# WeijingShi/Point-GNN

Measured on AMD Instinct MI355X. Metric: KITTI-shaped frames/sec (car_auto_T3 inference: graph build + GNN, 20000 pts/frame, mean E1 602k), higher is better.
Workload: dtype f32

## Files before the change

include/pointgnn_hip.h:

```cpp
#ifndef POINTGNN_HIP_H_
#define POINTGNN_HIP_H_

#include <stddef.h>
#include <stdint.h>

#ifdef __cplusplus
extern "C" {
#endif

#define PGNN_E_INVALID (-1)
#define PGNN_E_WORKSPACE (-2)
#define PGNN_E_UNSUPPORTED (-3)
#define PGNN_E_CAPACITY (-4)
#define PGNN_E_COMM (-5)

int pgnn_version(void);
const char *pgnn_last_error(void);
int pgnn_check_device_pointer(const void *device_ptr);

int pgnn_stream_create_cu_mask(int32_t cu_first, int32_t cu_count,
                               int32_t complement, void **stream_out);
int pgnn_stream_destroy(void *stream);

int pgnn_scatter_max_f32(const float *data, int64_t ld_data,
// ... 319 lines not shown
                                       int32_t num_vertices,
                                       const pgnn_fc_layer *layer_host,
                                       int32_t edges_sorted, float *out,
                                       int64_t ld_out, float *rows_out,
                                       int64_t ld_rows, float *h1_out,
                                       void *stream);

int pgnn_offset_apply(const float *xyz, const float *delta, int64_t ld_delta,
                      int64_t n_rows, const float *wx, float *xyz_out,
                      float *Q, int64_t ld_q, void *stream);

int pgnn_vertex_pre_edge_fwd(const float *h, int64_t ld_h, int32_t c,
                             const float *xyz,
                             const pgnn_fc_layer *offset_layers_host,
                             int32_t n_offset_layers,
                             const pgnn_fc_layer *p_layer_host, const float *wx,
                             int64_t n_vertices, float *P, float *Q,
                             int64_t ld_pq, float *agg, int64_t ld_agg,
                             void *stream);
int pgnn_vertex_pre_edge_fwd_dyn(const float *h, int64_t ld_h, int32_t c,
                                 const float *xyz,
                                 const pgnn_fc_layer *offset_layers_host,
                                 int32_t n_offset_layers,
                                 const pgnn_fc_layer *p_layer_host,
                                 const float *wx, int64_t vertices_cap,
                                 float *P, float *Q, int64_t ld_pq, float *agg,
                                 int64_t ld_agg,
                                 const pgnn_dyn_count *n_vertices,
                                 void *stream);

int pgnn_vertex_update_pre_edge_fwd(
    const float *x, int64_t ld_x, int32_t nx,
    const pgnn_fc_layer *front_layers_host, int32_t n_front,
    const float *residual, int64_t ld_res, float *y, int64_t ld_y, int32_t c,
    const float *xyz, const pgnn_fc_layer *offset_layers_host,
    int32_t n_offset_layers, const pgnn_fc_layer *p_layer_host, const float *wx,
    int64_t n_vertices, float *P, float *Q, int64_t ld_pq, float *agg,
    int64_t ld_agg, void *stream);
int pgnn_vertex_update_pre_edge_fwd_dyn(
    const float *x, int64_t ld_x, int32_t nx,
    const pgnn_fc_layer *front_layers_host, int32_t n_front,
    const float *residual, int64_t ld_res, float *y, int64_t ld_y, int32_t c,
    const float *xyz, const pgnn_fc_layer *offset_layers_host,
    int32_t n_offset_layers, const pgnn_fc_layer *p_layer_host, const float *wx,
    int64_t vertices_cap, float *P, float *Q, int64_t ld_pq, float *agg,
    int64_t ld_agg, const pgnn_dyn_count *n_vertices, void *stream);

int pgnn_mlp2_fwd(const float *x, int64_t ld_x, int32_t nx,
                  const pgnn_fc_layer *front_layers_host, int32_t n_front,
                  const float *residual, int64_t ld_res, float *y, int64_t ld_y,
                  int32_t ny, const pgnn_fc_layer *back_layers_host,
                  int32_t n_back, float *out, int64_t ld_out, int64_t n_rows,
                  void *stream);
int pgnn_mlp2_fwd_dyn(const float *x, int64_t ld_x, int32_t nx,
                      const pgnn_fc_layer *front_layers_host, int32_t n_front,
                      const float *residual, int64_t ld_res, float *y,
                      int64_t ld_y, int32_t ny,
                      const pgnn_fc_layer *back_layers_host, int32_t n_back,
                      float *out, int64_t ld_out, int64_t rows_cap,
                      const pgnn_dyn_count *rows, void *stream);


int pgnn_pack_fc_device(const float *w, const float *b, int32_t k_in,
                        int32_t n_out, int32_t transpose, float *packed,
                        void *stream);

int pgnn_pack_fc_many(const void *jobs_device, int32_t n_jobs,
                      int32_t total_blocks, void *stream);

int pgnn_edge_hidden_fwd(const float *P, const float *Q, int64_t ld_pq,
                         const int32_t *edges, int64_t n_edges, float *H1,
                         void *stream);
int pgnn_edge_hidden_bwd(const float *dH1, int64_t ld, const int32_t *edges,
                         int64_t n_edges, int64_t n_vertices, float *dP,
                         float *dQ, void *stream);
typedef struct pgnn_merge_job {
  const void *src;
  void *dst;
  int64_t n_words;
  int32_t add0, add1;
} pgnn_merge_job;
int pgnn_merge_rows(const pgnn_merge_job *jobs_host, int32_t n_jobs,
                    void *stream);
int pgnn_pool_features_fwd(const float *point_features, int32_t n_feat,
                           const float *point_xyz,
                           const int32_t *keypoint_indices,
                           const int32_t *edges, int64_t n_edges, float *F,
                           void *stream);
int pgnn_pool_features_wide_fwd(const float *point_features,
                                int64_t ld_features, int32_t n_feat,
                                const float *point_xyz,
                                const int32_t *keypoint_indices,
                                const int32_t *edges, int64_t n_edges, float *F,
                                int64_t ld_f, void *stream);
int pgnn_relu_mask_mul(float *dY, const float *Y, int64_t count, void *stream);
int pgnn_scatter_max_bwd_f32(const float *data, int64_t ld_data,
                             const int32_t *seg_ids, int64_t n_rows,
                             int32_t n_cols, int32_t num_segments,
                             const float *out, int64_t ld_out,
                             const float *grad_out, int64_t ld_grad_out,
                             int32_t *tie_count_ws, float *grad_data,
                             int64_t ld_grad_data, int32_t relu_mask,
                             void *stream);
size_t pgnn_segmax_fc_bwd_workspace_bytes(int64_t n_rows, int32_t n_cols,
                                          int32_t num_segments, int32_t k_in);
int pgnn_segmax_fc_bwd_f32(const float *Y, int64_t ld_y,
                           const int32_t *seg_ids, int64_t n_rows,
                           int32_t n_cols, int32_t num_segments,
                           const float *out, int64_t ld_out,
                           const float *grad_out, int64_t ld_go,
                           const float *X, int64_t ld_x, int32_t k_in,
                           const float *WT, int64_t ld_wt, float *dX,
                           int64_t ld_dx, int32_t dx_cols, int32_t mask_x,
                           float *dW, float *db, void *workspace,
                           size_t workspace_bytes, void *stream);
int pgnn_edge_segmax_fc_bwd_f32(const float *Y, int64_t ld_y,
                                const int32_t *edges, const int32_t *dst_ids,
                                int64_t n_edges, int32_t n_cols,
                                int32_t num_vertices, const float *out,
                                int64_t ld_out, const float *grad_out,
                                int64_t ld_go, const float *H1, int64_t ld_h1,
                                const float *P, const float *Q, int32_t k_in,
                                const float *WT, int64_t ld_wt,
                                float *dP, float *dQ, int64_t ld_pq, float *dW,
                                float *db, void *workspace,
                                size_t workspace_bytes, void *stream);
size_t pgnn_weight_grad_workspace_bytes(int32_t k_in, int32_t n_out,
                                        int64_t n_rows);
int pgnn_weight_grad_f32(const float *X, int64_t ld_x, int32_t k_in,
                         const float *dZ, int64_t ld_dz, int32_t n_out,
                         int64_t n_rows, float *dW, float *db,
                         int32_t accumulate, void *workspace,
                         size_t workspace_bytes, void *stream);
size_t pgnn_pool_narrow_bwd_workspace_bytes(int64_t n_rows);
int pgnn_pool_narrow_bwd_f32(const float *feat, const float *act0,
                             const float *act1, const float *dz2,
                             int64_t n_rows, const float *w2t_packed,
                             const float *w1t_packed, int32_t k_in0, float *dW0,
                             float *db0, float *dW1, float *db1, float *dW2,
                             float *db2, int32_t accumulate, void *workspace,
                             size_t workspace_bytes, void *stream);
typedef struct pgnn_wgrad_job {
  const float *X;
  int64_t ld_x;
  const float *dZ;
  int64_t ld_dz;
  int64_t n_rows;
  float *dW;
  float *db;
  int32_t k_in, n_out;
  int32_t accumulate, reserved;
} pgnn_wgrad_job;
size_t pgnn_weight_grad_many_workspace_bytes(const pgnn_wgrad_job *jobs_host,
                                             int32_t n_jobs);
int pgnn_weight_grad_many_f32(const pgnn_wgrad_job *jobs_host, int32_t n_jobs,
                              void *workspace, size_t workspace_bytes,
                              void *stream);
int pgnn_loss_fwd_bwd(const float *logits, int64_t ld_logits,
                      const int32_t *labels, const float *pred_box,
                      int32_t box_len, const float *gt_box, const float *valid,
                      int64_t n_vertices, int32_t num_classes,
                      float cls_grad_scale, float loc_grad_scale,
                      double *sums4, float *dlogits, float *dpred_box,
                      void *stream);
int pgnn_loss_fwd_bwd_counts(const float *logits, int64_t ld_logits,
                             const int32_t *labels, const float *pred_box,
// ... 123 lines not shown
                              int32_t num_classes, int32_t *out_index,
                              int32_t *out_label, int64_t capacity,
                              int32_t *out_count, void *stream);
int pgnn_detection_candidates_dyn(const float *probs, int64_t n_vertices_cap,
                                  const int32_t *n_vertices_dev,
                                  int32_t num_classes, int32_t *out_index,
                                  int32_t *out_label, int64_t capacity,
                                  int32_t *out_count, void *stream);
size_t pgnn_nms_workspace_bytes(int64_t n_boxes);
int pgnn_nms_boxes_3d(const int32_t *class_labels, const float *boxes_3d,
                      const float *scores, const int32_t *attributes,
                      int64_t n_boxes, double overlapped_thres, int32_t mode,
                      float appr_factor, int64_t top_k, void *workspace,
                      size_t workspace_bytes, int32_t *out_labels,
                      float *out_boxes, float *out_scores,
                      int32_t *out_attributes, int32_t *out_count,
                      void *stream);
int pgnn_overlapped_boxes_3d(const float *single_box, const float *boxes_3d,
                             int64_t n_boxes, float appr_factor,
                             double *overlap, void *stream);
int pgnn_overlapped_boxes_3d_raster(const int32_t *single_box_corners,
                                    const int32_t *box_corners, int64_t n_boxes,
                                    double *overlap, void *stream);

int pgnn_assign_box_labels(const float *xyz, int64_t n_points,
                           const double *label_records, int32_t n_records,
                           int32_t *cls_labels, double *boxes_3d,
                           float *valid_boxes, int32_t *owner, void *stream);
int pgnn_assign_box_labels_f64(const double *xyz, int64_t n_points,
                               const double *label_records, int32_t n_records,
                               int32_t *cls_labels, double *boxes_3d,
                               float *valid_boxes, int32_t *owner,
                               void *stream);
int pgnn_box_encode_f64(const int32_t *cls_labels, const float *xyz,
                        const double *boxes, const double *class_table,
                        int32_t n_table, int64_t n_rows, int32_t boxes_per_row,
                        float *encoded, void *stream);
int pgnn_box_encode_f64_xyz64(const int32_t *cls_labels, const double *xyz,
                              const double *boxes, const double *class_table,
                              int32_t n_table, int64_t n_rows,
                              int32_t boxes_per_row, float *encoded,
                              void *stream);

int pgnn_points_affine_f64(double *xyz, int64_t n_points, const double *rot_3x3,
                           const double *shift_3, const int32_t *select,
                           void *stream);
int pgnn_points_in_box_f64(const double *xyz, int64_t n_points,
                           const double *box_record_24, const int32_t *exclude,
                           int32_t *inside, int32_t *count, void *stream);

size_t pgnn_metrics_state_bytes(int32_t n_classes, int32_t n_thresholds);
int pgnn_metrics_update(const float *probs, int64_t ld_probs,
                        const int32_t *labels, int64_t n_rows,
                        int32_t n_classes, int32_t n_thresholds, void *state,
                        void *stream);
int pgnn_metrics_compute(const void *state, int32_t n_classes,
                         int32_t n_thresholds, float *out, void *stream);

size_t pgnn_kitti_ingest_workspace_bytes(int64_t n_points);
int pgnn_kitti_cam_points_in_image(
    const float *velo_points, int64_t n_points, const float *velo_to_cam_3x4,
    const double *cam_to_image_3x3, double image_width, double image_height,
    const uint8_t *image_bgr, int64_t image_rows, int64_t image_cols,
    void *workspace, size_t workspace_bytes, float *out_xyz, float *out_attr,
    int32_t attr_dim, int64_t capacity, int32_t *out_count, void *stream);

size_t pgnn_voxel_average_workspace_bytes(int64_t n_points, int32_t attr_dim);
int pgnn_voxel_average_f32(const float *xyz, const float *attr,
                           int32_t attr_dim, int64_t n_points,
                           const int32_t *n_dev, double voxel_size,
                           void *workspace, size_t workspace_bytes,
                           double *out_xyz, double *out_attr, int32_t *out_lens,
                           int64_t capacity, int32_t *out_count, void *stream);
size_t pgnn_kitti_cam_points_voxel_in_image_workspace_bytes(int64_t n_points);
int pgnn_kitti_cam_points_voxel_in_image(
    const float *velo_points, int64_t n_points, const float *velo_to_cam_3x4,
    const double *cam_to_image_3x3, double image_width, double image_height,
    const uint8_t *image_bgr, int64_t image_rows, int64_t image_cols,
    double voxel_size, void *workspace, size_t workspace_bytes,
    double *out_xyz, double *out_attr, int32_t attr_dim, int64_t capacity,
    int32_t *out_count, void *stream);

int pgnn_set_tunable(const char *key, int value);
int pgnn_set_debug_buffer(void *device_ptr);

#ifdef __cplusplus
}
#endif
#endif
```

point-gnn_amd/_lib.py:

```python
import ctypes
import os

import torch

_HERE = os.path.dirname(os.path.abspath(__file__))
LIB_PATH = os.environ.get("PGNN_LIB") or os.path.join(_HERE, "libpointgnn_hip.so")

c_i32, c_i64, c_f64 = ctypes.c_int32, ctypes.c_int64, ctypes.c_double
c_vp, c_sz, c_u64 = ctypes.c_void_p, ctypes.c_size_t, ctypes.c_uint64

PGNN_MAX_LAYERS = 8


class FcLayer(ctypes.Structure):
    _fields_ = [("packed", c_vp), ("k_in", c_i32), ("n_out", c_i32),
                ("relu_from", c_i32)]


class DynCount(ctypes.Structure):
    _fields_ = [("dev", c_vp), ("hint", c_i64)]


class WgradJob(ctypes.Structure):
    _fields_ = [("X", c_vp), ("ld_x", c_i64), ("dZ", c_vp), ("ld_dz", c_i64),
                ("n_rows", c_i64), ("dW", c_vp), ("db", c_vp), ("k_in", c_i32),
                ("n_out", c_i32), ("accumulate", c_i32), ("reserved", c_i32)]


class MergeJob(ctypes.Structure):
    _fields_ = [("src", c_vp), ("dst", c_vp), ("n_words", c_i64),
                ("add0", c_i32), ("add1", c_i32)]


class PackJob(ctypes.Structure):
    _fields_ = [("w", c_vp), ("b", c_vp), ("dst", c_vp), ("k_in", c_i32),
                ("n_out", c_i32), ("kind", c_i32), ("first_block", c_i32),
                ("ld", c_i32), ("reserved", c_i32)]


TRAIN_MAX_FC, TRAIN_MAX_STAGES, TRAIN_MAX_CLASSES, TRAIN_MAX_LEVELS = 8, 8, 16, 4


class TrainFc(ctypes.Structure):
    _fields_ = [("w_off", c_i64), ("b_off", c_i64), ("k_in", c_i32),
                ("n_out", c_i32)]


class TrainStage(ctypes.Structure):
    _fields_ = [("kind", c_i32), ("graph_level", c_i32), ("n_a", c_i32),
                ("n_b", c_i32), ("n_c", c_i32), ("reserved", c_i32),
                ("a", TrainFc * TRAIN_MAX_FC), ("b", TrainFc * TRAIN_MAX_FC),
                ("c", TrainFc * TRAIN_MAX_FC)]


class TrainModel(ctypes.Structure):
    _fields_ = [("n_stages", c_i32), ("num_classes", c_i32),
                ("box_len", c_i32), ("reserved", c_i32), ("n_params", c_i64),
                ("stages", TrainStage * TRAIN_MAX_STAGES),
                ("cls", TrainFc * 2),
                ("loc", (TrainFc * 3) * TRAIN_MAX_CLASSES)]


class TrainBatch(ctypes.Structure):
    _fields_ = [("input_v", c_vp), ("n_feat", c_i32), ("n_levels", c_i32),
                ("n_vertices", c_i64 * (TRAIN_MAX_LEVELS + 1)),
                ("coords", c_vp * (TRAIN_MAX_LEVELS + 1)),
                ("keypoints", c_vp * TRAIN_MAX_LEVELS),
                ("edges", c_vp * TRAIN_MAX_LEVELS),
                ("n_edges", c_i64 * TRAIN_MAX_LEVELS),
                ("edges_sorted", c_i32 * TRAIN_MAX_LEVELS)]


class PointGnnHipError(RuntimeError):
    pass


_SIGNATURES = {
    "pgnn_version": (c_i32, []),
    "pgnn_last_error": (ctypes.c_char_p, []),
    "pgnn_stream_create_cu_mask": (c_i32, [c_i32, c_i32, c_i32,
                                           ctypes.POINTER(c_vp)]),
    "pgnn_stream_destroy": (c_i32, [c_vp]),
    "pgnn_check_device_pointer": (c_i32, [c_vp]),
    "pgnn_set_tunable": (c_i32, [ctypes.c_char_p, c_i32]),
    "pgnn_set_debug_buffer": (c_i32, [c_vp]),
    "pgnn_scatter_max_f32": (c_i32, [c_vp, c_i64, c_vp, c_i64, c_i32, c_i32,
                                     c_vp, c_i64, c_i32, c_vp]),
    "pgnn_scatter_sum_f32": (c_i32, [c_vp, c_i64, c_vp, c_i64, c_i32, c_i32,
                                     c_vp, c_i64, c_i32, c_vp, c_vp]),
    "pgnn_radius_graph_workspace_bytes": (c_sz, [c_i64, c_i64]),
    "pgnn_radius_graph_count": (c_i32, [c_vp, c_i64, c_vp, c_i64, c_f64, c_vp,
                                        c_vp, c_sz, c_vp, c_vp]),
    "pgnn_radius_graph_fill": (c_i32, [c_vp, c_i64, c_vp, c_i64, c_f64, c_vp,
                                       c_vp, c_sz, c_vp, c_vp, c_i64, c_vp]),
    "pgnn_radius_graph_count_f64": (c_i32, [c_vp, c_i64, c_vp, c_i64, c_f64,
                                            c_vp, c_vp, c_sz, c_vp, c_vp]),
    "pgnn_radius_graph_fill_f64": (c_i32, [c_vp, c_i64, c_vp, c_i64, c_f64,
                                           c_vp, c_vp, c_sz, c_vp, c_vp, c_i64,
                                           c_vp]),
    "pgnn_radius_graph_dyn_workspace_bytes": (c_sz, [c_i64, c_i64]),
    "pgnn_radius_graph_dyn": (c_i32, [c_vp, c_i64, c_vp, c_vp, c_i64, c_vp,
                                      c_f64, c_vp, c_vp, c_sz, c_vp, c_i64,
                                      c_vp, c_vp]),
    "pgnn_radius_graph_dyn_f64": (c_i32, [c_vp, c_i64, c_vp, c_vp, c_i64, c_vp,
                                          c_f64, c_vp, c_vp, c_sz, c_vp, c_i64,
                                          c_vp, c_vp]),
    "pgnn_radius_graph_dyn_grid": (c_i32, [c_vp, c_i64, c_vp, c_i64, c_f64,
                                           c_vp, c_vp, c_sz, c_vp]),
    "pgnn_radius_graph_dyn_grid_f64": (c_i32, [c_vp, c_i64, c_vp, c_i64, c_f64,
                                               c_vp, c_vp, c_sz, c_vp]),
    "pgnn_radius_graph_dyn_query": (c_i32, [c_vp, c_i64, c_vp, c_i64, c_vp,
                                            c_f64, c_vp, c_vp, c_sz, c_vp,
                                            c_i64, c_vp, c_vp]),
    "pgnn_radius_graph_dyn_query_f64": (c_i32, [c_vp, c_i64, c_vp, c_i64, c_vp,
# ... 133 lines not shown
        c_i32, c_vp, c_i64, c_vp, ctypes.POINTER(DynCount),
        ctypes.POINTER(DynCount), c_vp]),
    "pgnn_pack_fc_f16x2_acc": (c_i32, [c_vp, c_vp, c_i32, c_i32, c_vp]),
    "pgnn_point_set_pooling_f16x2_fwd": (c_i32, [
        c_vp, c_i32, c_vp, c_vp, c_vp, c_i64, c_i32, ctypes.POINTER(FcLayer),
        c_i32, c_vp, c_vp, c_i32, c_vp, c_i64, c_vp, c_vp, ctypes.POINTER(DynCount),
        ctypes.POINTER(DynCount), c_vp]),
    "pgnn_offset_apply": (c_i32, [c_vp, c_vp, c_i64, c_i64, c_vp, c_vp, c_vp,
                                  c_i64, c_vp]),
    "pgnn_vertex_pre_edge_fwd": (c_i32, [c_vp, c_i64, c_i32, c_vp,
                                         ctypes.POINTER(FcLayer), c_i32,
                                         ctypes.POINTER(FcLayer), c_vp, c_i64,
                                         c_vp, c_vp, c_i64, c_vp, c_i64,
                                         c_vp]),
    "pgnn_vertex_update_pre_edge_fwd": (c_i32, [
        c_vp, c_i64, c_i32, ctypes.POINTER(FcLayer), c_i32, c_vp, c_i64, c_vp,
        c_i64, c_i32, c_vp, ctypes.POINTER(FcLayer), c_i32,
        ctypes.POINTER(FcLayer), c_vp, c_i64, c_vp, c_vp, c_i64, c_vp, c_i64,
        c_vp]),
    "pgnn_vertex_update_pre_edge_fwd_dyn": (c_i32, [
        c_vp, c_i64, c_i32, ctypes.POINTER(FcLayer), c_i32, c_vp, c_i64, c_vp,
        c_i64, c_i32, c_vp, ctypes.POINTER(FcLayer), c_i32,
        ctypes.POINTER(FcLayer), c_vp, c_i64, c_vp, c_vp, c_i64, c_vp, c_i64,
        ctypes.POINTER(DynCount), c_vp]),
    "pgnn_mlp2_fwd": (c_i32, [
        c_vp, c_i64, c_i32, ctypes.POINTER(FcLayer), c_i32, c_vp, c_i64, c_vp,
        c_i64, c_i32, ctypes.POINTER(FcLayer), c_i32, c_vp, c_i64, c_i64,
        c_vp]),
    "pgnn_mlp2_fwd_dyn": (c_i32, [
        c_vp, c_i64, c_i32, ctypes.POINTER(FcLayer), c_i32, c_vp, c_i64, c_vp,
        c_i64, c_i32, ctypes.POINTER(FcLayer), c_i32, c_vp, c_i64, c_i64,
        ctypes.POINTER(DynCount), c_vp]),
    "pgnn_pack_fc_device": (c_i32, [c_vp, c_vp, c_i32, c_i32, c_i32, c_vp,
                                    c_vp]),
    "pgnn_pack_fc_many": (c_i32, [c_vp, c_i32, c_i32, c_vp]),
    "pgnn_segmax_fc_bwd_workspace_bytes": (c_sz, [c_i64, c_i32, c_i32, c_i32]),
    "pgnn_edge_segmax_fc_bwd_f32": (c_i32, [c_vp, c_i64, c_vp, c_vp, c_i64,
                                            c_i32, c_i32, c_vp, c_i64, c_vp,
                                            c_i64, c_vp, c_i64, c_vp, c_vp,
                                            c_i32, c_vp, c_i64, c_vp, c_vp,
                                            c_i64, c_vp, c_vp, c_vp, c_sz,
                                            c_vp]),
    "pgnn_segmax_fc_bwd_f32": (c_i32, [c_vp, c_i64, c_vp, c_i64, c_i32, c_i32,
                                       c_vp, c_i64, c_vp, c_i64, c_vp, c_i64,
                                       c_i32, c_vp, c_i64, c_vp, c_i64, c_i32,
                                       c_i32, c_vp, c_vp, c_vp, c_sz, c_vp]),
    "pgnn_trainer_create": (c_i32, [ctypes.POINTER(TrainModel),
                                    ctypes.POINTER(c_vp)]),
    "pgnn_trainer_destroy": (c_i32, [c_vp]),
    "pgnn_trainer_images_bytes": (c_sz, [c_vp]),
    "pgnn_trainer_bind": (c_i32, [c_vp, c_vp, c_vp, c_vp, c_sz, c_vp]),
    "pgnn_trainer_repack": (c_i32, [c_vp, c_vp]),
    "pgnn_trainer_workspace_bytes": (c_sz, [c_vp, ctypes.POINTER(TrainBatch)]),
    "pgnn_trainer_forward": (c_i32, [c_vp, ctypes.POINTER(TrainBatch), c_vp,
                                     c_sz, ctypes.POINTER(c_vp),
                                     ctypes.POINTER(c_i64),
                                     ctypes.POINTER(c_vp), c_vp]),
    "pgnn_trainer_backward": (c_i32, [c_vp, ctypes.POINTER(TrainBatch), c_vp,
                                      c_sz, c_vp, c_vp, c_vp]),
    "pgnn_trainer_backward_sync": (c_i32, [c_vp, ctypes.POINTER(TrainBatch),
                                           c_vp, c_sz, c_vp, c_vp, c_vp, c_vp,
                                           c_i64, c_vp]),
    "pgnn_comm_unique_id": (c_i32, [c_vp]),
    "pgnn_comm_init_rank": (c_i32, [c_vp, c_i32, c_i32, ctypes.POINTER(c_vp)]),
    "pgnn_comm_destroy": (c_i32, [c_vp]),
    "pgnn_comm_info": (c_i32, [c_vp, ctypes.POINTER(c_i32),
                               ctypes.POINTER(c_i32), ctypes.POINTER(c_i32)]),
    "pgnn_comm_library": (ctypes.c_char_p, []),
    "pgnn_comm_async_error": (c_i32, [c_vp]),
    "pgnn_allreduce_sum_f32": (c_i32, [c_vp, c_vp, c_i64, c_vp]),
    "pgnn_allreduce_sum_f64": (c_i32, [c_vp, c_vp, c_i64, c_vp]),
    "pgnn_allreduce_step": (c_i32, [c_vp, c_vp, c_i64, c_vp, c_i64, c_vp]),
    "pgnn_broadcast_f32": (c_i32, [c_vp, c_vp, c_i64, c_i32, c_vp]),
    "pgnn_edge_hidden_fwd": (c_i32, [c_vp, c_vp, c_i64, c_vp, c_i64, c_vp,
                                     c_vp]),
    "pgnn_edge_hidden_bwd": (c_i32, [c_vp, c_i64, c_vp, c_i64, c_i64, c_vp,
                                     c_vp, c_vp]),
    "pgnn_pool_features_wide_fwd": (c_i32, [c_vp, c_i64, c_i32, c_vp, c_vp, c_vp,
                                            c_i64, c_vp, c_i64, c_vp]),
    "pgnn_pool_features_fwd": (c_i32, [c_vp, c_i32, c_vp, c_vp, c_vp, c_i64,
                                       c_vp, c_vp]),
    "pgnn_relu_mask_mul": (c_i32, [c_vp, c_vp, c_i64, c_vp]),
    "pgnn_merge_rows": (c_i32, [ctypes.POINTER(MergeJob), c_i32, c_vp]),
    "pgnn_scatter_max_bwd_f32": (c_i32, [c_vp, c_i64, c_vp, c_i64, c_i32,
                                         c_i32, c_vp, c_i64, c_vp, c_i64, c_vp,
                                         c_vp, c_i64, c_i32, c_vp]),
    "pgnn_weight_grad_workspace_bytes": (c_sz, [c_i32, c_i32, c_i64]),
    "pgnn_weight_grad_f32": (c_i32, [c_vp, c_i64, c_i32, c_vp, c_i64, c_i32,
                                     c_i64, c_vp, c_vp, c_i32, c_vp, c_sz,
                                     c_vp]),
    "pgnn_weight_grad_many_workspace_bytes": (c_sz,
                                              [ctypes.POINTER(WgradJob),
                                               c_i32]),
    "pgnn_weight_grad_many_f32": (c_i32, [ctypes.POINTER(WgradJob), c_i32,
                                          c_vp, c_sz, c_vp]),
    "pgnn_pool_narrow_bwd_workspace_bytes": (c_sz, [c_i64]),
    "pgnn_pool_narrow_bwd_f32": (c_i32, [c_vp, c_vp, c_vp, c_vp, c_i64, c_vp,
                                         c_vp, c_i32, c_vp, c_vp, c_vp, c_vp,
                                         c_vp, c_vp, c_i32, c_vp, c_sz, c_vp]),
    "pgnn_loss_fwd_bwd": (c_i32, [c_vp, c_i64, c_vp, c_vp, c_i32, c_vp, c_vp,
                                  c_i64, c_i32, ctypes.c_float, ctypes.c_float,
                                  c_vp, c_vp, c_vp, c_vp]),
    "pgnn_loss_fwd_bwd_counts": (c_i32, [c_vp, c_i64, c_vp, c_vp, c_i32, c_vp,
                                         c_vp, c_i64, c_i32, ctypes.c_double,
                                         ctypes.c_double, c_vp, c_vp, c_vp,
                                         c_vp, c_vp]),
    "pgnn_loss_fwd_bwd_ex": (c_i32, [c_vp, c_i64, c_vp, c_vp, c_i32, c_vp, c_vp,
                                     c_i64, c_i32, ctypes.c_float,
                                     ctypes.c_float, c_vp, ctypes.c_double,
                                     ctypes.c_double, c_i32, ctypes.c_float,
                                     ctypes.c_float, c_vp, c_vp, c_vp, c_vp,
                                     c_vp]),
    "pgnn_loss_fwd_bwd_sel": (c_i32, [c_vp, c_i64, c_vp, c_vp, c_i32, c_vp,
                                      c_vp, c_i64, c_i32, ctypes.c_float,
                                      ctypes.c_float, c_vp, ctypes.c_double,
                                      ctypes.c_double, c_i32, ctypes.c_float,
                                      ctypes.c_float, c_vp, c_vp, c_vp,
                                      ctypes.c_float, c_vp, c_vp, c_vp, c_vp,
                                      c_vp, c_vp]),
    "pgnn_topk_mask_workspace_bytes": (c_sz, [c_i64]),
    "pgnn_topk_mask_f32": (c_i32, [c_vp, c_i64, c_i64, c_vp, c_vp, c_sz, c_vp]),
    "pgnn_sgd_step": (c_i32, [c_vp, c_vp, c_vp, c_i64, ctypes.c_float,
                              ctypes.c_float, ctypes.c_float, c_vp]),
    "pgnn_optimizer_step": (c_i32, [c_i32, c_vp, c_vp, c_vp, c_vp, c_vp, c_i64] +
                            [ctypes.c_float] * 6 + [c_vp]),
    "pgnn_l1_norm": (c_i32, [c_vp, c_vp, c_i64, c_vp, c_vp]),
    "pgnn_box_decode_f32": (c_i32, [c_vp, c_vp, c_vp, c_vp, c_i32, c_i64,
                                    c_i32, c_vp, c_vp]),
    "pgnn_box_encode_f32": (c_i32, [c_vp, c_vp, c_vp, c_vp, c_i32, c_i64,
                                    c_i32, c_vp, c_vp]),
    "pgnn_detection_candidates": (c_i32, [c_vp, c_i64, c_i32, c_vp, c_vp,
                                          c_i64, c_vp, c_vp]),
    "pgnn_detection_candidates_dyn": (c_i32, [c_vp, c_i64, c_vp, c_i32, c_vp,
                                              c_vp, c_i64, c_vp, c_vp]),
    "pgnn_nms_workspace_bytes": (c_sz, [c_i64]),
    "pgnn_nms_boxes_3d": (c_i32, [c_vp, c_vp, c_vp, c_vp, c_i64,
                                  c_f64, c_i32, ctypes.c_float, c_i64,
                                  c_vp, c_sz, c_vp, c_vp, c_vp, c_vp, c_vp,
                                  c_vp]),
    "pgnn_overlapped_boxes_3d": (c_i32, [c_vp, c_vp, c_i64, ctypes.c_float,
                                         c_vp, c_vp]),
    "pgnn_overlapped_boxes_3d_raster": (c_i32, [c_vp, c_vp, c_i64, c_vp,
                                                c_vp]),
    "pgnn_assign_box_labels": (c_i32, [c_vp, c_i64, c_vp, c_i32, c_vp, c_vp,
                                       c_vp, c_vp, c_vp]),
    "pgnn_assign_box_labels_f64": (c_i32, [c_vp, c_i64, c_vp, c_i32, c_vp,
                                           c_vp, c_vp, c_vp, c_vp]),
    "pgnn_box_encode_f64": (c_i32, [c_vp, c_vp, c_vp, c_vp, c_i32, c_i64,
                                    c_i32, c_vp, c_vp]),
    "pgnn_box_encode_f64_xyz64": (c_i32, [c_vp, c_vp, c_vp, c_vp, c_i32, c_i64,
                                          c_i32, c_vp, c_vp]),
    "pgnn_points_affine_f64": (c_i32, [c_vp, c_i64, c_vp, c_vp, c_vp, c_vp]),
    "pgnn_points_in_box_f64": (c_i32, [c_vp, c_i64, c_vp, c_vp, c_vp, c_vp,
                                       c_vp]),
    "pgnn_kitti_ingest_workspace_bytes": (c_sz, [c_i64]),
    "pgnn_kitti_cam_points_in_image": (c_i32, [c_vp, c_i64, c_vp, c_vp, c_f64,
                                               c_f64, c_vp, c_i64, c_i64, c_vp,
                                               c_sz, c_vp, c_vp, c_i32, c_i64,
                                               c_vp, c_vp]),
    "pgnn_voxel_average_workspace_bytes": (c_sz, [c_i64, c_i32]),
    "pgnn_voxel_average_f32": (c_i32, [c_vp, c_vp, c_i32, c_i64, c_vp, c_f64,
                                       c_vp, c_sz, c_vp, c_vp, c_vp, c_i64,
                                       c_vp, c_vp]),
    "pgnn_kitti_cam_points_voxel_in_image_workspace_bytes": (c_sz, [c_i64]),
    "pgnn_kitti_cam_points_voxel_in_image": (
        c_i32, [c_vp, c_i64, c_vp, c_vp, c_f64, c_f64, c_vp, c_i64, c_i64,
# ... 32 lines not shown
    if _lib is not None:
        return _lib
    if not os.path.exists(LIB_PATH) and not os.environ.get("PGNN_LIB"):
        _build_missing()
    if not os.path.exists(LIB_PATH):
        raise PointGnnHipError(
            "libpointgnn_hip.so not found at %s -- the HIP extension is "
            "required (no CPU fallback); run `python -m pointgnn_amd.build`"
            % LIB_PATH)
    lib = ctypes.CDLL(LIB_PATH)
    for name, (res, args) in _SIGNATURES.items():
        fn = getattr(lib, name)
        fn.restype = res
        fn.argtypes = args
    _lib = lib
    for kv in filter(None, os.environ.get("PGNN_TUNE", "").split(",")):
        k, v = kv.split("=")
        check(lib.pgnn_set_tunable(k.strip().encode(), int(v)),
              "PGNN_TUNE " + kv)
    return lib


E_INVALID = -1
E_WORKSPACE = -2
E_UNSUPPORTED = -3
AGG_MAX, AGG_SUM, AGG_MEAN = 0, 1, 2


def check(rc, what=""):
    if rc != 0:
        msg = load().pgnn_last_error()
        raise PointGnnHipError("%s failed (code %d): %s" % (
            what or "pgnn call", rc, msg.decode() if msg else "?"))


_SCHED_WS = {}
SCHED_WS_INTS = 64


def sched_ws(device=None):
    import torch
    dev = torch.device("cuda", torch.cuda.current_device()) \
        if device is None or device.index is None else device
    key = (dev.index, torch.cuda.current_stream(dev).cuda_stream)
    t = _SCHED_WS.get(key)
    if t is None:
        t = _SCHED_WS[key] = torch.zeros(SCHED_WS_INTS, dtype=torch.int32,
                                         device=dev)
    return t


def stream_ptr():
    return ctypes.c_void_p(torch.cuda.current_stream().cuda_stream)


def ptr(t):
    if t is None:
        return ctypes.c_void_p(0)
    return ctypes.c_void_p(t.data_ptr())


class DeviceCount(object):
    __slots__ = ("dev", "hint", "frame")

    def __init__(self, dev, hint=0, frame=None):
        self.dev = dev
        self.hint = int(hint)
        self.frame = frame

    def arg(self):
        return ctypes.byref(DynCount(self.dev.data_ptr(), self.hint))


def tag_count(t, count):
    if count is not None:
        t._pgnn_count = count
    return t


def count_of(t):
    return getattr(t, "_pgnn_count", None) if t is not None else None


def set_tunable(key, value):
    check(load().pgnn_set_tunable(key.encode(), int(value)), "pgnn_set_tunable")
```

point-gnn_amd/csrc/gnn.hip:

```cpp
#include "mlp_engine.h"
#include "edge_ws.h"
#include "edge_ws_split.h"
#include "pool_ws.h"
#include "pool_split.h"
#include "pool_ws_f16.h"

namespace pgnn {
int g_mlp_blocks_per_cu = 4;
int g_edge_msub = 0;
int g_pool_msub = 0;
int g_mlp_pool_pct = 12;
int g_ws_xcds = 8;
int g_ws_prio = 1;
int g_f16_pool = 1;
int g_b16_force = 0;
int g_ws_pool_pct = 0;
int g_ws_chunk = 2;
int g_ws_balance = 1;
int g_ws_reserve = 0;
void *g_mlp_ts = nullptr;
int g_mlp_debug = 0;
}

namespace {
using namespace pgnn;

enum { PRO_ROWS = 0, PRO_POOL = 1, PRO_EDGE = 2,
       PRO_POOL_R3 = 3 };
constexpr bool is_pool(int pro) { return pro == PRO_POOL || pro == PRO_POOL_R3; }
constexpr bool is_pool_reg(int pro) { return pro == PRO_POOL_R3; }
constexpr int kMaxRegisterRuns = 6;

struct RowsArgs {
  const float *x;
  int64_t ldx;
  int nx;
  const float *x2;
  int64_t ldx2;
  int nx2;
  const float *res;
  int64_t ldres;
  float *y;
  int64_t ldy;
  int res_gate;
  float *mid[PGNN_MAX_LAYERS - 1];
  const float *gate[PGNN_MAX_LAYERS - 1];
};
struct PoolArgs {
  const float *feat;
  int nfeat;
  const float *xyz;
  const int32_t *kp;
  const int32_t *edges;
  int reg_hidden;
};
struct EdgeArgs {
  const float *P;
  const float *Q;
  int64_t ldpq;
  const int32_t *edges;
};
struct SegArgs {
  float *out;
  int64_t ldo;
  int num_segments;
  int sorted;
};

__host__ __device__ inline int ints_bytes(int rows) {
  return ((2 * rows + 2) * 4 + 15) / 16 * 16;
}

struct CarryState {
  int id;
  int left_closed;
};

__device__ __forceinline__ CarryState carry_after(unsigned long long starts,
                                                  int myd, int d_before,
                                                  int d_after, const SegArgs &sa,
                                                  CarryState cs, bool keep_open) {
  CarryState out = {-1, 0};
// ... 19 lines not shown
  const int myd = lane < ROWS ? dst[lane + 1] : -2;
  const int prevd = lane < ROWS ? dst[lane] : -2;
  const unsigned long long starts =
      __ballot(lane < ROWS && (lane == 0 || myd != prevd));
  const int d_before = dst[0], d_after = dst[ROWS + 1];
  for (int c = threadIdx.x; c < ncols; c += 256) {
    const float *col = stT + c * ROWS;
    const int sw = c & SWZ;
    v4f x[G];
#pragma unroll
    for (int g = 0; g < G; ++g)
      x[g] = *reinterpret_cast<const v4f *>(col + ((g ^ sw) << 2));
    unsigned long long rem = starts;
    while (rem) {
      const int r = __builtin_ctzll(rem);
      rem &= rem - 1;
      const int re = rem ? __builtin_ctzll(rem) : ROWS;
      const int d = __builtin_amdgcn_readlane(myd, r);
      if (d >= 0 && d < sa.num_segments) {
        bool left_closed = (r > 0) || (d_before != d);
        const bool merge = sa.sorted && r == 0 && cs.id == d;
        if (merge) left_closed = cs.left_closed != 0;
        const bool right_closed = (re < ROWS) || (d_after != d);
        const bool defer = sa.sorted && !right_closed && keep_open;
        const bool whole = sa.sorted && left_closed && right_closed;
        const int g0 = r >> 2, g1 = (re - 1) >> 2;
        float m = kFloatLowest;
#pragma unroll
        for (int g = 0; g < G; ++g) {
          if (g > g0 && g < g1) {
            m = fmaxf(fmaxf(m, x[g][0]), fmaxf(x[g][1], fmaxf(x[g][2], x[g][3])));
          } else if (g == g0 || g == g1) {
#pragma unroll
            for (int i = 0; i < 4; ++i) {
              const int row = 4 * g + i;
              if (row >= r && row < re) m = fmaxf(m, x[g][i]);
            }
          }
        }
        if (merge) m = fmaxf(m, carry[col0 + c]);
        if (defer) {
          carry[col0 + c] = m;
        } else {
          float *o = sa.out + (int64_t)d * sa.ldo + col0 + c;
          if (whole)
            *o = m;
          else
            atomic_max_f32(o, m + 0.0f);
        }
      }
    }
  }
  return carry_after(starts, myd, d_before, d_after, sa, cs, keep_open);
}

template <int ROWS>
__device__ __forceinline__ void consume_rows(const float *__restrict__ stage,
                                             int ld, int64_t row0, int rows_valid,
                                             int col0, int ncols,
                                             const RowsArgs &ra) {
  const int total = rows_valid * ncols;
  for (int idx = threadIdx.x; idx < total; idx += blockDim.x) {
    const int r = idx / ncols, c = idx - r * ncols;
    float v = stage[r * ld + c];
    if (ra.res) {
      const float a = ra.res[(row0 + r) * ra.ldres + col0 + c];
      v = ra.res_gate ? (a > 0.0f ? v : 0.0f) : v + a;
    }
    ra.y[(row0 + r) * ra.ldy + col0 + c] = v;
  }
}

__device__ __forceinline__ int opaque_lane(int lane_id) {
  int lane;
  asm volatile("v_mov_b32 %0, %1" : "=v"(lane) : "v"(lane_id));
  return lane;
}

constexpr int kRowSteps = 10;

__device__ __forceinline__ void consume_rows16(const float *__restrict__ stage,
                                               int ld, int64_t row0,
                                               int rows_valid, int col0,
                                               int ncols, const RowsArgs &ra) {
  const int r = threadIdx.x >> 5, c0 = threadIdx.x & 31;
  const int64_t row = row0 + (r < rows_valid ? r : rows_valid - 1);
  float add[kRowSteps];
  if (ra.res) {
    const float *__restrict__ rr = ra.res + row * ra.ldres + col0;
#pragma unroll
    for (int j = 0; j < kRowSteps; ++j) {
      const int c = c0 + 32 * j;
      add[j] = rr[c < ncols ? c : ncols - 1];
    }
  }
  float *__restrict__ yr = ra.y + row * ra.ldy + col0;
#pragma unroll
  for (int j = 0; j < kRowSteps; ++j) {
    const int c = c0 + 32 * j;
    if (r < rows_valid && c < ncols) {
      float v = stage[r * ld + c];
      if (ra.res) v = ra.res_gate ? (add[j] > 0.0f ? v : 0.0f) : v + add[j];
      yr[c] = v;
    }
  }
}

__device__ __forceinline__ void tap_rows16(float *tile, int ld, int64_t row0,
                                           int rows_valid, int ncols,
                                           const float *__restrict__ gate,
                                           float *__restrict__ mid) {
  const int r = threadIdx.x >> 5, c0 = threadIdx.x & 31;
  const int64_t row = row0 + (r < rows_valid ? r : rows_valid - 1);
  for (int cb = 0; cb < ncols; cb += 32 * kRowSteps) {
    const int left = ncols - cb;
    float g[kRowSteps];
    if (gate) {
      const float *__restrict__ gr = gate + row * ncols + cb;
#pragma unroll
      for (int j = 0; j < kRowSteps; ++j) {
        const int c = c0 + 32 * j;
        g[j] = gr[c < left ? c : left - 1];
      }
    }
    float *tr = tile + r * ld + cb;
    float *__restrict__ mr = mid ? mid + row * ncols + cb : nullptr;
#pragma unroll
    for (int j = 0; j < kRowSteps; ++j) {
      const int c = c0 + 32 * j;
      if (c < left) {
        float v = tr[c];
        if (gate) {
          v = g[j] > 0.0f ? v : 0.0f;
          tr[c] = v;
        }
        if (mr && r < rows_valid) mr[c] = v;
      }
    }
  }
  if (gate) __syncthreads();
}

__device__ __forceinline__ void load_rows16(const float *__restrict__ x,
                                            int64_t ldx, int nx, float *tile,
                                            int ld0, int kc, int64_t row0,
                                            int rows_valid) {
  const int r = threadIdx.x >> 5, c0 = threadIdx.x & 31;
  const float *__restrict__ xr =
      x + (row0 + (r < rows_valid ? r : rows_valid - 1)) * ldx;
  for (int cb = 0; cb < kc; cb += 32 * kRowSteps) {
    float v[kRowSteps];
#pragma unroll
    for (int j = 0; j < kRowSteps; ++j) {
      const int c = cb + c0 + 32 * j;
      v[j] = xr[c < nx ? c : nx - 1];
    }
#pragma unroll
    for (int j = 0; j < kRowSteps; ++j) {
      const int c = cb + c0 + 32 * j;
      if (c < kc) tile[r * ld0 + c] = (r < rows_valid && c < nx) ? v[j] : 0.0f;
    }
  }
}

template <int MSUB, int PRO>
__global__ __launch_bounds__(256, 2) void fused_mlp_kernel(
    ChainDev chain, int64_t n_rows, RowsArgs ra, PoolArgs pa, EdgeArgs ea,
    SegArgs sa, int stage_off ,
    int dbg, long long *ts ,
    int32_t *sched ,
    int64_t n_static ,
    const int32_t *n_dev ,
    int dyn_pool_pct ) {
  constexpr int ROWS = 16 * MSUB;
  if (n_dev) {
    const int64_t nd = *n_dev;
    n_rows = nd < n_rows ? nd : n_rows;
  }
#ifndef PGNN_DIAG
  dbg &= ~7;
#endif
  extern __shared__ __attribute__((aligned(16))) char smem[];
  int *dst = reinterpret_cast<int *>(smem);
  float *part = reinterpret_cast<float *>(dst + ROWS + 2);
  if (MSUB == 4 && threadIdx.x < 48) part[threadIdx.x] = kFloatLowest;
  float *carry = reinterpret_cast<float *>(smem + ints_bytes(ROWS));
  float *tile = carry + 16 * chain.l[chain.n - 1].nt;
  float *stage = stage_off >= 0 ? tile + stage_off : tile;
  const int lane = threadIdx.x & 63;
  const int wave = __builtin_amdgcn_readfirstlane(threadIdx.x >> 6);
  const int64_t n_tiles = (n_rows + ROWS - 1) / ROWS;
  const int ld0 = lds_ld(16 * chain.l[0].kq);

  if (n_dev) {
    if (sched && n_tiles >= 6 * (int64_t)gridDim.x)
      n_static = n_tiles - n_tiles * dyn_pool_pct / 100;
    else
      sched = nullptr;
  }
  if (!sched) n_static = n_tiles;
  const int64_t tq = n_static / gridDim.x, trem = n_static % gridDim.x;
  const int64_t tile_first =
      blockIdx.x * tq + (blockIdx.x < trem ? blockIdx.x : trem);
  int64_t tile_last = tile_first + tq + (blockIdx.x < trem ? 1 : 0);
  __shared__ int s_claim;
  CarryState cs = {-1, 0};
  int nxt_s = 0, nxt_d = -1, nxt_k = 0;
  bool fresh = true;
  int tile_seq = 0;
  for (int64_t tile_id = tile_first;; ++tile_id, ++tile_seq) {
    if (tile_id >= tile_last) {
      if (tile_id >= n_tiles || !sched) break;
      if (threadIdx.x == 0)
        s_claim = __hip_atomic_fetch_add(&sched[0], 1, __ATOMIC_RELAXED,
                                         __HIP_MEMORY_SCOPE_AGENT);
      __syncthreads();
      tile_id = n_static + __builtin_amdgcn_readfirstlane(s_claim);
      if (tile_id >= n_tiles) break;
      tile_last = tile_id + 1;
      cs.id = -1;
      cs.left_closed = 0;
      fresh = true;
    }
    const int64_t row0 = tile_id * ROWS;
    const int rows_valid =
        (int)((n_rows - row0 < ROWS) ? (n_rows - row0) : ROWS);
    long long *tsp = nullptr;
    if (ts && tile_seq < 32 && threadIdx.x == 0) {
      tsp = ts + ((int64_t)blockIdx.x * 32 + tile_seq) * 8;
      tsp[0] = __builtin_readcyclecounter();
// ... 387 lines not shown
int make_plan(const pgnn_fc_layer *layers, int32_t n_layers, int first_k,
              Plan &p) {
  PGNN_REQUIRE(layers && n_layers >= 1 && n_layers <= PGNN_MAX_LAYERS,
               PGNN_E_INVALID, "mlp: 1..PGNN_MAX_LAYERS layers required");
  p.chain.n = n_layers;
  int prev_nt = -1;
  int max_ld = 0;
  for (int i = 0; i < n_layers; ++i) {
    const pgnn_fc_layer &l = layers[i];
    PGNN_REQUIRE(l.packed && l.k_in > 0 && l.n_out > 0, PGNN_E_INVALID,
                 "mlp: bad layer");
    LayerDev &d = p.chain.l[i];
    d.wp = l.packed;
    d.kq = (l.k_in + 15) / 16;
    d.nt = (l.n_out + 15) / 16;
    d.relu_from = l.relu_from;
    if (i == 0) {
      PGNN_REQUIRE(first_k <= l.k_in, PGNN_E_INVALID,
                   "mlp: input wider than first layer");
    } else {
      PGNN_REQUIRE(d.kq == prev_nt, PGNN_E_INVALID,
                   "mlp: layer widths do not chain");
    }
    if (i + 1 < n_layers)
      PGNN_REQUIRE(d.nt <= kMaxTilesPerPass, PGNN_E_UNSUPPORTED,
                   "mlp: hidden width > 320 not supported");
    prev_nt = d.nt;
    const int ld_in = lds_ld(16 * d.kq);
    if (ld_in > max_ld) max_ld = ld_in;
    if (i + 1 < n_layers || d.nt <= kMaxTilesPerPass) {
      const int ld_out = lds_ld(16 * d.nt);
      if (ld_out > max_ld) max_ld = ld_out;
    }
  }
  p.tile_floats_per_row = max_ld;
  p.stage_cols =
      p.chain.l[n_layers - 1].nt > kMaxTilesPerPass ? 16 * kMaxTilesPerPass : 0;
  return 0;
}

size_t plan_lds_bytes(const Plan &p, int rows) {
  size_t floats = (size_t)rows * p.tile_floats_per_row;
  floats += 16 * (size_t)p.chain.l[p.chain.n - 1].nt;
  if (p.stage_cols) floats += (size_t)rows * lds_ld(p.stage_cols);
  return ints_bytes(rows) + floats * 4;
}

template <int MSUB, int PRO>
int launch_fused(const Plan &p, int64_t n_rows, const RowsArgs &ra,
                 const PoolArgs &pa, const EdgeArgs &ea, const SegArgs &sa,
                 hipStream_t stream, int32_t *sched = nullptr,
                 const int32_t *n_dev = nullptr) {
  constexpr int ROWS = 16 * MSUB;
  const size_t lds = plan_lds_bytes(p, ROWS);
  PGNN_REQUIRE(lds <= 160 * 1024, PGNN_E_UNSUPPORTED,
               "mlp: layer too wide for the LDS tile");
  auto kern = fused_mlp_kernel<MSUB, PRO>;
  const int64_t n_tiles = (n_rows + ROWS - 1) / ROWS;
  int per_cu = (int)((160 * 1024) / lds);
  if (per_cu > g_mlp_blocks_per_cu) per_cu = g_mlp_blocks_per_cu;
  if (per_cu < 1) per_cu = 1;
  int64_t grid = (int64_t)stream_cu_count(stream) * per_cu;
  if (grid > n_tiles) grid = n_tiles;
  int64_t n_static = n_tiles;
  if (g_mlp_ts || g_mlp_pool_pct <= 0 || (!n_dev && n_tiles < 6 * grid))
    sched = nullptr;
  if (sched) n_static = n_tiles - n_tiles * g_mlp_pool_pct / 100;
  PGNN_HIP((hipError_t)arm_sched(sched, stream));
  const int stage_off = p.stage_cols ? ROWS * p.tile_floats_per_row : -1;
  if (g_mlp_debug & 16) {
    int nb = -1;
    hipError_t e = hipOccupancyMaxActiveBlocksPerMultiprocessor(
        &nb, reinterpret_cast<const void *>(kern), 256, lds);
    fprintf(stderr, "[pgnn] fused<%d,%d> lds=%zu per_cu=%d occupancy_api=%d (%d) grid=%lld tiles=%lld\n",
            MSUB, PRO, lds, per_cu, nb, (int)e, (long long)grid, (long long)n_tiles);
  }
  return launch_lds(kern, dim3((unsigned)grid), dim3(256), lds, stream, p.chain,
                    n_rows, ra, pa, ea, sa, stage_off, g_mlp_debug,
                    (long long *)g_mlp_ts, sched, n_static, n_dev,
                    g_mlp_pool_pct);
}

constexpr int kRowsWaves = 8;

template <bool TAPS>
__global__ __launch_bounds__(64 * kRowsWaves) void rows_mlp_kernel(
    ChainDev chain, int64_t n_rows, RowsArgs ra, int stage_off,
    const int32_t *n_dev ) {
  constexpr int ROWS = 16, NW = kRowsWaves;
  if (n_dev) {
    const int64_t nd = *n_dev;
    n_rows = nd < n_rows ? nd : n_rows;
  }
  extern __shared__ __attribute__((aligned(16))) char smem[];
  float *tile = reinterpret_cast<float *>(smem);
  float *stage = stage_off >= 0 ? tile + stage_off : tile;
  const int lane_id = threadIdx.x & 63;
  const int wave = __builtin_amdgcn_readfirstlane(threadIdx.x >> 6);
  const int64_t n_tiles = (n_rows + ROWS - 1) / ROWS;
  const int ld0 = lds_ld(16 * chain.l[0].kq);
  for (int64_t tile_id = blockIdx.x; tile_id < n_tiles; tile_id += gridDim.x) {
    const int lane = opaque_lane(lane_id);
    const int64_t row0 = tile_id * ROWS;
    const int rows_valid =
        (int)((n_rows - row0 < ROWS) ? (n_rows - row0) : ROWS);
    const int kc = 16 * chain.l[0].kq;
    KrowPre pre;
    krow_prefetch(chain.l[0], 0, wave, lane, pre);
    if (ra.nx2 == 0) {
      static_assert(64 * NW == 32 * ROWS, "one 32-thread group per row");
      load_rows16(ra.x, ra.ldx, ra.nx, tile, ld0, kc, row0, rows_valid);
    } else {
    for (int idx = threadIdx.x; idx < ROWS * kc; idx += 64 * NW) {
      const int r = idx / kc, c = idx - r * kc;
      float v = 0.0f;
      if (r < rows_valid) {
        if (c < ra.nx)
          v = ra.x[(row0 + r) * ra.ldx + c];
        else if (c < ra.nx + ra.nx2)
          v = ra.x2[(row0 + r) * ra.ldx2 + (c - ra.nx)];
      }
      tile[r * ld0 + c] = v;
    }
    }
    __syncthreads();
    for (int li = 0; li + 1 < chain.n; ++li) {
      const LayerDev &L = chain.l[li];
      krow_pass(tile, lds_ld(16 * L.kq), tile, lds_ld(16 * L.nt), L, 0, wave,
                lane, pre, true, chain.l[li + 1], 0);
      if constexpr (TAPS)
        tap_rows16(tile, lds_ld(16 * L.nt), row0, rows_valid, 16 * L.nt,
                   ra.gate[li], ra.mid[li]);
    }
    const LayerDev &L = chain.l[chain.n - 1];
    const int ld_in = lds_ld(16 * L.kq);
    for (int t0 = 0; t0 < L.nt; t0 += kMaxTilesPerPass) {
      int tiles = L.nt - t0;
      if (tiles > kMaxTilesPerPass) tiles = kMaxTilesPerPass;
      const int ncols = 16 * tiles;
      const int ld_st = lds_ld(ncols);
      const bool more = t0 + kMaxTilesPerPass < L.nt;
      krow_pass(tile, ld_in, stage, ld_st, L, t0, wave, lane, pre, more, L,
                t0 + kMaxTilesPerPass);
      consume_rows16(stage, ld_st, row0, rows_valid, 16 * t0, ncols, ra);
      __syncthreads();
    }
  }
}

template <bool TAPS = false>
int launch_rows8(const Plan &p, int64_t n_rows, const RowsArgs &ra,
                 hipStream_t stream, const int32_t *n_dev = nullptr,
                 int64_t grid_tiles = 0 ) {
  const size_t lds = plan_lds_bytes(p, 16);
  PGNN_REQUIRE(lds <= 160 * 1024, PGNN_E_UNSUPPORTED,
               "mlp: layer too wide for the LDS tile");
  const int64_t n_tiles = (n_rows + 15) / 16;
  const int stage_off = p.stage_cols ? 16 * p.tile_floats_per_row : -1;
  return launch_lds(rows_mlp_kernel<TAPS>,
                    dim3((unsigned)(grid_tiles > 0 ? grid_tiles : n_tiles)),
                    dim3(64 * kRowsWaves), lds, stream, p.chain, n_rows, ra,
                    stage_off, n_dev);
}

int fill_lowest(float *out, int64_t count, hipStream_t stream) {
  PGNN_HIP(hipMemsetD32Async((hipDeviceptr_t)out, (int)kFloatLowestBits,
// ... 679 lines not shown
    const pgnn_dyn_count *n_edges, const pgnn_dyn_count *num_vertices,
    int32_t aggregation, void *workspace, size_t workspace_bytes,
    void *stream_) {
  PGNN_GUARD_BEGIN
  PGNN_REQUIRE(n_edges && n_edges->dev && num_vertices && num_vertices->dev,
               PGNN_E_INVALID, "edge_mlp_agg_dyn: null count");
  return edge_agg_impl(P, Q, ld_pq, width, edges, edges_cap, vertices_cap, layers,
                       n_layers, edges_sorted, out, ld_out, sched_ws, aggregation,
                       workspace, workspace_bytes, (hipStream_t)stream_,
                       dyn_of(n_edges), dyn_of(num_vertices), true, nullptr);
  PGNN_GUARD_END
}

extern "C" int pgnn_point_set_pooling_agg_workspace_bytes(
    const pgnn_fc_layer *layers, int32_t n_layers, int32_t n_feat,
    int64_t edges_cap, int64_t edges_hint, int32_t keypoints_cap,
    int32_t aggregation, int32_t capacity_form, void *stream_, size_t *bytes) {
  PGNN_GUARD_BEGIN
  PGNN_REQUIRE(bytes && layers, PGNN_E_INVALID,
               "pooling_agg_workspace_bytes: bad arguments");
  const int64_t n_sel =
      (capacity_form && edges_hint > 0 && edges_hint < edges_cap) ? edges_hint
                                                                  : edges_cap;
  return pooling_agg_impl(nullptr, n_feat, nullptr, nullptr, nullptr, n_sel,
                          keypoints_cap, layers, n_layers, 0, nullptr, 0, nullptr,
                          aggregation, nullptr, 0, (hipStream_t)stream_,
                          dyn_of(nullptr), dyn_of(nullptr), capacity_form != 0,
                          bytes);
  PGNN_GUARD_END
}

extern "C" int pgnn_point_set_pooling_agg_fwd(
    const float *point_features, int32_t n_feat, const float *point_xyz,
    const int32_t *keypoint_indices, const int32_t *edges, int64_t n_edges,
    int32_t num_keypoints, const pgnn_fc_layer *layers, int32_t n_layers,
    int32_t edges_sorted, float *out, int64_t ld_out, int32_t *sched_ws,
    int32_t aggregation, void *workspace, size_t workspace_bytes,
    void *stream_) {
  PGNN_GUARD_BEGIN
  return pooling_agg_impl(point_features, n_feat, point_xyz, keypoint_indices,
                          edges, n_edges, num_keypoints, layers, n_layers,
                          edges_sorted, out, ld_out, sched_ws, aggregation,
                          workspace, workspace_bytes, (hipStream_t)stream_,
                          dyn_of(nullptr), dyn_of(nullptr), false, nullptr);
  PGNN_GUARD_END
}

extern "C" int pgnn_point_set_pooling_agg_fwd_dyn(
    const float *point_features, int32_t n_feat, const float *point_xyz,
    const int32_t *keypoint_indices, const int32_t *edges, int64_t edges_cap,
    int32_t keypoints_cap, const pgnn_fc_layer *layers, int32_t n_layers,
    int32_t edges_sorted, float *out, int64_t ld_out, int32_t *sched_ws,
    const pgnn_dyn_count *n_edges, const pgnn_dyn_count *num_keypoints,
    int32_t aggregation, void *workspace, size_t workspace_bytes,
    void *stream_) {
  PGNN_GUARD_BEGIN
  PGNN_REQUIRE(n_edges && n_edges->dev && num_keypoints && num_keypoints->dev,
               PGNN_E_INVALID, "pooling_agg_dyn: null count");
  return pooling_agg_impl(point_features, n_feat, point_xyz, keypoint_indices,
                          edges, edges_cap, keypoints_cap, layers, n_layers,
                          edges_sorted, out, ld_out, sched_ws, aggregation,
                          workspace, workspace_bytes, (hipStream_t)stream_,
                          dyn_of(n_edges), dyn_of(num_keypoints), true, nullptr);
  PGNN_GUARD_END
}

namespace {

struct PreEdgeArgs {
  const float *h;
  int64_t ld_h;
  int c;
  const float *xyz;
  const float *wx;
  int64_t n;
  const int32_t *n_dev;
  float *P, *Q;
  int64_t ld_pq;
  float *agg;
  int64_t ld_agg;
  int ld_tile, ld_scratch;
};

__device__ __forceinline__ void pre_edge_tail(const ChainDev &off,
                                              const LayerDev &pl,
                                              const PreEdgeArgs &a, float *tile,
                                              float *scratch, float *stage,
                                              int64_t row0, int rows_valid,
                                              int wave, int lane, KrowPre &pre) {
  const float *delta = nullptr;
  int ld_delta = 0;
  for (int li = 0; li < off.n; ++li) {
    const LayerDev &L = off.l[li];
    const float *in = li == 0 ? tile : scratch;
    const int ld_in = li == 0 ? a.ld_tile : lds_ld(16 * L.kq);
    krow_pass(in, ld_in, scratch, lds_ld(16 * L.nt), L, 0, wave, lane, pre,
              true, li + 1 < off.n ? off.l[li + 1] : pl, 0);
    delta = scratch;
    ld_delta = lds_ld(16 * L.nt);
  }
  {
    const int r = threadIdx.x >> 5, c0 = threadIdx.x & 31;
    const int ldq = (int)a.ld_pq;
    const int64_t row = row0 + (r < rows_valid ? r : rows_valid - 1);
    float x0 = a.xyz[row * 3], x1 = a.xyz[row * 3 + 1], x2 = a.xyz[row * 3 + 2];
    float w0[kRowSteps], w1[kRowSteps], w2[kRowSteps];
#pragma unroll
    for (int j = 0; j < kRowSteps; ++j) {
      const int c = c0 + 32 * j;
      const int cc = c < ldq ? c : ldq - 1;
      w0[j] = a.wx[cc];
      w1[j] = a.wx[ldq + cc];
      w2[j] = a.wx[2 * ldq + cc];
    }
    if (delta) {
      x0 = x0 + delta[r * ld_delta];
      x1 = x1 + delta[r * ld_delta + 1];
      x2 = x2 + delta[r * ld_delta + 2];
    }
    float *__restrict__ qr = a.Q + row * a.ld_pq;
#pragma unroll
    for (int j = 0; j < kRowSteps; ++j) {
      const int c = c0 + 32 * j;
      if (r < rows_valid && c < ldq)
        qr[c] = (x0 * w0[j] + x1 * w1[j]) + x2 * w2[j];
    }
  }
  const int ld_st = lds_ld(16 * pl.nt);
  krow_pass(tile, a.ld_tile, stage, ld_st, pl, 0, wave, lane, pre, false, pl, 0);
  RowsArgs ra = {};
  ra.y = a.P;
  ra.ldy = a.ld_pq;
  consume_rows16(stage, ld_st, row0, rows_valid, 0, 16 * pl.nt, ra);
}

template <bool STRIDE>
__global__ __launch_bounds__(64 * kRowsWaves) void vertex_pre_edge_kernel(
    ChainDev off, LayerDev pl, PreEdgeArgs a) {
  constexpr int ROWS = 16;
  extern __shared__ __attribute__((aligned(16))) char smem[];
  float *tile = reinterpret_cast<float *>(smem);
  float *scratch = tile + ROWS * a.ld_tile;
  float *stage = scratch + ROWS * a.ld_scratch;
  const int lane_id = threadIdx.x & 63;
  const int wave = __builtin_amdgcn_readfirstlane(threadIdx.x >> 6);
  int64_t n_rows = a.n;
  if (a.n_dev) {
    const int64_t nd = *a.n_dev;
    n_rows = nd < n_rows ? nd : n_rows;
  }
  for (int64_t row0 = (int64_t)blockIdx.x * ROWS; row0 < n_rows;
       row0 += STRIDE ? (int64_t)gridDim.x * ROWS : n_rows) {
    const int lane = opaque_lane(lane_id);
  const int rows_valid =
      (int)((n_rows - row0 < ROWS) ? (n_rows - row0) : ROWS);
  const int kc = 16 * pl.kq;
  KrowPre pre;
  krow_prefetch(off.n > 0 ? off.l[0] : pl, 0, wave, lane, pre);
  {
    static_assert(64 * kRowsWaves == 32 * ROWS, "one 32-thread group per row");
    const int r = threadIdx.x >> 5, c0 = threadIdx.x & 31;
    const int64_t rowc = row0 + (r < rows_valid ? r : rows_valid - 1);
    const float *__restrict__ hr = a.h + rowc * a.ld_h;
    const float *__restrict__ xr = a.xyz + rowc * 3;
    for (int cb = 0; cb < kc; cb += 32 * kRowSteps) {
      float v[kRowSteps];
#pragma unroll
      for (int j = 0; j < kRowSteps; ++j) {
        const int c = cb + c0 + 32 * j;
        const int d = c - a.c;
        const float hv = hr[c < a.c ? c : a.c - 1];
        const float xv = xr[d < 0 ? 0 : (d > 2 ? 2 : d)];
        v[j] = c < a.c ? hv : xv;
      }
#pragma unroll
      for (int j = 0; j < kRowSteps; ++j) {
        const int c = cb + c0 + 32 * j;
        if (c < kc)
          tile[r * a.ld_tile + c] =
              (r < rows_valid && c < a.c + 3) ? v[j] : 0.0f;
      }
    }
  }
  if (a.agg) {
    for (int idx = threadIdx.x; idx < rows_valid * (int)a.ld_agg; idx += 64 * kRowsWaves)
      a.agg[row0 * a.ld_agg + idx] = kFloatLowest;
  }
  __syncthreads();
  pre_edge_tail(off, pl, a, tile, scratch, stage, row0, rows_valid, wave, lane,
                pre);
  if (STRIDE) __syncthreads();
  }
}

struct FrontArgs {
  const float *x;
  int64_t ldx;
  int nx;
  const float *res;
  int64_t ldres;
  float *y;
  int64_t ldy;
  int ld_buf;
  int ld_stage;
  long long *ts;
};

__device__ __forceinline__ void front_chain(const ChainDev &front, float *tile,
                                            float *stage, int ld_stage,
                                            int wave, int lane, KrowPre &pre,
                                            const LayerDev after,
                                            long long *tsw, int &n_stamp) {
  for (int li = 0; li + 1 < front.n; ++li) {
    const LayerDev &L = front.l[li];
    krow_pass(tile, lds_ld(16 * L.kq), tile, lds_ld(16 * L.nt), L, 0, wave,
              lane, pre, true, front.l[li + 1], 0);
    if (tsw && n_stamp < 14) {
      const long long cyc = __builtin_readcyclecounter();
      if (threadIdx.x == 0) tsw[n_stamp] = cyc;
      ++n_stamp;
    }
  }
  const LayerDev &L = front.l[front.n - 1];
  krow_pass(tile, lds_ld(16 * L.kq), stage, ld_stage, L, 0, wave, lane, pre,
            true, after, 0);
}

template <bool STRIDE>
__global__ __launch_bounds__(64 * kRowsWaves) void vertex_update_pre_edge_kernel(
    ChainDev front, FrontArgs f, ChainDev off, LayerDev pl, PreEdgeArgs a) {
  constexpr int ROWS = 16;
  static_assert(64 * kRowsWaves == 32 * ROWS, "one 32-thread group per row");
  extern __shared__ __attribute__((aligned(16))) char smem[];
  float *tile = reinterpret_cast<float *>(smem);
  float *scratch = tile + ROWS * f.ld_buf;
  float *stage = scratch + ROWS * a.ld_scratch;
  const int lane_id = threadIdx.x & 63;
  const int wave = __builtin_amdgcn_readfirstlane(threadIdx.x >> 6);
  int64_t n_rows = a.n;
  if (a.n_dev) {
    const int64_t nd = *a.n_dev;
    n_rows = nd < n_rows ? nd : n_rows;
  }
  const int kc0 = 16 * front.l[0].kq;
  const int ncols_y = 16 * front.l[front.n - 1].nt;
  const int kc = 16 * pl.kq;
  long long *tsw = f.ts ? f.ts + (int64_t)blockIdx.x * 16 : nullptr;
  int n_stamp = 0;
  auto stamp = [&]() {
    if (tsw && n_stamp < 15) {
      __builtin_amdgcn_sched_barrier(0);
      const long long cyc = __builtin_readcyclecounter();
      if (threadIdx.x == 0) tsw[n_stamp] = cyc;
      ++n_stamp;
      __builtin_amdgcn_sched_barrier(0);
    }
  };
  if (tsw && threadIdx.x == 0) tsw[15] = __builtin_amdgcn_s_memrealtime();
  for (int64_t row0 = (int64_t)blockIdx.x * ROWS; row0 < n_rows;
       row0 += STRIDE ? (int64_t)gridDim.x * ROWS : n_rows) {
    const int lane = opaque_lane(lane_id);
    const int rows_valid =
        (int)((n_rows - row0 < ROWS) ? (n_rows - row0) : ROWS);
    stamp();
    KrowPre pre;
    krow_prefetch(front.l[0], 0, wave, lane, pre);
    load_rows16(f.x, f.ldx, f.nx, tile, lds_ld(kc0), kc0, row0, rows_valid);
    if (a.agg) {
      for (int idx = threadIdx.x; idx < rows_valid * (int)a.ld_agg;
           idx += 64 * kRowsWaves)
        a.agg[row0 * a.ld_agg + idx] = kFloatLowest;
    }
    __syncthreads();
    stamp();
    front_chain(front, tile, stage, f.ld_stage, wave, lane, pre,
                off.n > 0 ? off.l[0] : pl, tsw, n_stamp);
    stamp();
    {
      const int r = threadIdx.x >> 5, c0 = threadIdx.x & 31;
      const int64_t row = row0 + (r < rows_valid ? r : rows_valid - 1);
      float add[kRowSteps];
      if (f.res) {
        const float *__restrict__ rr = f.res + row * f.ldres;
#pragma unroll
        for (int j = 0; j < kRowSteps; ++j) {
          const int c = c0 + 32 * j;
          add[j] = rr[c < ncols_y ? c : ncols_y - 1];
        }
      }
      const float xv0 = a.xyz[row * 3], xv1 = a.xyz[row * 3 + 1],
                  xv2 = a.xyz[row * 3 + 2];
      float *__restrict__ yr = f.y + row * f.ldy;
#pragma unroll
      for (int j = 0; j < kRowSteps; ++j) {
        const int c = c0 + 32 * j;
        if (c < kc) {
          float v = 0.0f;
          if (r < rows_valid) {
            if (c < ncols_y) {
              float sv = stage[r * f.ld_stage + c];
              if (f.res) sv += add[j];
              yr[c] = sv;
              if (c < a.c) v = sv;
            }
            const int d = c - a.c;
            if (d >= 0 && d < 3) v = d == 0 ? xv0 : (d == 1 ? xv1 : xv2);
          }
          tile[r * a.ld_tile + c] = v;
        }
      }
    }
    __syncthreads();
    stamp();
    pre_edge_tail(off, pl, a, tile, scratch, stage, row0, rows_valid, wave, lane,
                  pre);
    stamp();
    if (STRIDE) __syncthreads();
  }
  if (tsw && threadIdx.x == 0) tsw[14] = __builtin_amdgcn_s_memrealtime();
}

template <bool STRIDE>
__global__ __launch_bounds__(64 * kRowsWaves) void vertex_mlp2_kernel(
    ChainDev front, FrontArgs f, ChainDev back, RowsArgs out, int64_t n_rows,
    const int32_t *n_dev) {
  constexpr int ROWS = 16;
  extern __shared__ __attribute__((aligned(16))) char smem[];
  float *tile = reinterpret_cast<float *>(smem);
  float *stage = tile + ROWS * f.ld_buf;
  const int lane_id = threadIdx.x & 63;
  const int wave = __builtin_amdgcn_readfirstlane(threadIdx.x >> 6);
  if (n_dev) {
    const int64_t nd = *n_dev;
    n_rows = nd < n_rows ? nd : n_rows;
  }
  const int kc0 = 16 * front.l[0].kq;
  const int ncols_y = 16 * front.l[front.n - 1].nt;
  const int kcb = 16 * back.l[0].kq;
  const int ld_b = lds_ld(kcb);
  for (int64_t row0 = (int64_t)blockIdx.x * ROWS; row0 < n_rows;
       row0 += STRIDE ? (int64_t)gridDim.x * ROWS : n_rows) {
    const int lane = opaque_lane(lane_id);
    const int rows_valid =
        (int)((n_rows - row0 < ROWS) ? (n_rows - row0) : ROWS);
    KrowPre pre;
    krow_prefetch(front.l[0], 0, wave, lane, pre);
    load_rows16(f.x, f.ldx, f.nx, tile, lds_ld(kc0), kc0, row0, rows_valid);
    __syncthreads();
    int no_stamp = 0;
    front_chain(front, tile, stage, f.ld_stage, wave, lane, pre, back.l[0],
                nullptr, no_stamp);
    const int kmax = kcb > ncols_y ? kcb : ncols_y;
    {
      const int r = threadIdx.x >> 5, c0 = threadIdx.x & 31;
      const int64_t row = row0 + (r < rows_valid ? r : rows_valid - 1);
      float add[kRowSteps];
      if (f.res) {
        const float *__restrict__ rr = f.res + row * f.ldres;
#pragma unroll
        for (int j = 0; j < kRowSteps; ++j) {
          const int c = c0 + 32 * j;
          add[j] = rr[c < ncols_y ? c : ncols_y - 1];
        }
      }
      float *__restrict__ yr = f.y + row * f.ldy;
#pragma unroll
      for (int j = 0; j < kRowSteps; ++j) {
        const int c = c0 + 32 * j;
        if (c < kmax) {
          float v = 0.0f;
          if (r < rows_valid && c < ncols_y) {
            float sv = stage[r * f.ld_stage + c];
            if (f.res) sv += add[j];
            yr[c] = sv;
            if (c < out.nx) v = sv;
          }
          if (c < kcb) tile[r * ld_b + c] = v;
        }
      }
    }
    __syncthreads();
    for (int li = 0; li + 1 < back.n; ++li) {
      const LayerDev &L = back.l[li];
      krow_pass(tile, lds_ld(16 * L.kq), tile, lds_ld(16 * L.nt), L, 0, wave,
                lane, pre, true, back.l[li + 1], 0);
    }
    const LayerDev &L = back.l[back.n - 1];
    const int ld_st = lds_ld(16 * L.nt);
    krow_pass(tile, lds_ld(16 * L.kq), stage, ld_st, L, 0, wave, lane, pre,
              false, L, 0);
    consume_rows16(stage, ld_st, row0, rows_valid, 0, 16 * L.nt, out);
    if (STRIDE) __syncthreads();
  }
}

}

namespace {
int plan_pre_edge(const char *name, int32_t c, const float *xyz,
                  const pgnn_fc_layer *offset_layers, int32_t n_offset_layers,
                  const pgnn_fc_layer *p_layer, const float *wx,
                  int64_t n_vertices, float *P, float *Q, int64_t ld_pq,
                  float *agg, int64_t ld_agg, const Dyn &dk, int kq_max,
                  ChainDev &off, LayerDev &pl, PreEdgeArgs &a) {
  const auto msg = [name](const char *what) { return std::string(name) + what; };
  Plan pp;
  int rc = make_plan(p_layer, 1, c + 3, pp);
  if (rc) return rc;
  pl = pp.chain.l[0];
  PGNN_REQUIRE(p_layer->k_in == c + 3 && pl.nt <= kMaxTilesPerPass &&
                   ld_pq == 16 * pl.nt,
               PGNN_E_INVALID,
               msg(": P layer must be [c+3 -> n], ld_pq = padded n").c_str());
  PGNN_REQUIRE(kq_max == 0 || pl.kq <= kq_max, PGNN_E_UNSUPPORTED,
               msg(": more than 317 features").c_str());
  off = {};
  int scratch_ld = lds_ld(16);
  if (n_offset_layers > 0) {
    Plan po;
    rc = make_plan(offset_layers, n_offset_layers, c, po);
    if (rc) return rc;
    off = po.chain;
    PGNN_REQUIRE(offset_layers[0].k_in == c &&
                     offset_layers[n_offset_layers - 1].n_out >= 3 &&
                     off.l[0].kq <= pl.kq &&
                     off.l[n_offset_layers - 1].nt <= kMaxTilesPerPass,
                 PGNN_E_INVALID,
                 msg(": offset chain must be [c -> ... -> 3]").c_str());
    for (int i = 0; i < n_offset_layers; ++i) {
      const int ld = lds_ld(16 * off.l[i].nt);
      if (ld > scratch_ld) scratch_ld = ld;
      if (i > 0 && lds_ld(16 * off.l[i].kq) > scratch_ld)
        scratch_ld = lds_ld(16 * off.l[i].kq);
    }
  }
  a.c = c;
  a.xyz = xyz;
  a.wx = wx;
  a.n = n_vertices;
  a.n_dev = dk.dev;
  a.P = P;
  a.Q = Q;
  a.ld_pq = ld_pq;
  a.agg = agg;
  a.ld_agg = ld_agg;
  a.ld_tile = lds_ld(16 * pl.kq);
  a.ld_scratch = scratch_ld;
  return 0;
}

int pre_edge_impl(
    const float *h, int64_t ld_h, int32_t c, const float *xyz,
    const pgnn_fc_layer *offset_layers, int32_t n_offset_layers,
    const pgnn_fc_layer *p_layer, const float *wx, int64_t n_vertices, float *P,
    float *Q, int64_t ld_pq, float *agg, int64_t ld_agg, hipStream_t stream,
    const Dyn &dk) {
  PGNN_REQUIRE(n_vertices >= 0 && c > 0 && ld_h >= c && n_offset_layers >= 0 &&
                   n_offset_layers <= PGNN_MAX_LAYERS && p_layer,
               PGNN_E_INVALID, "vertex_pre_edge: bad argument");
  if (n_vertices == 0) return 0;
  PGNN_REQUIRE(h && xyz && wx && P && Q && (!agg || ld_agg > 0), PGNN_E_INVALID,
               "vertex_pre_edge: null pointer");
  ChainDev off;
  LayerDev pl;
  PreEdgeArgs a;
  const int rc = plan_pre_edge("vertex_pre_edge", c, xyz, offset_layers,
                               n_offset_layers, p_layer, wx, n_vertices, P, Q,
                               ld_pq, agg, ld_agg, dk, 0, off, pl, a);
  if (rc) return rc;
  a.h = h;
  a.ld_h = ld_h;
  const size_t lds =
      (size_t)16 * (a.ld_tile + a.ld_scratch + lds_ld(16 * pl.nt)) * 4;
  PGNN_REQUIRE(lds <= 160 * 1024, PGNN_E_UNSUPPORTED,
               "vertex_pre_edge: layer too wide for the LDS tile");
  return launch_lds(
      dk.dev ? vertex_pre_edge_kernel<true> : vertex_pre_edge_kernel<false>,
      dim3((unsigned)dyn_grid_tiles(dk, n_vertices)), dim3(64 * kRowsWaves), lds,
      stream, off, pl, a);
}
}

namespace {
int plan_front(const float *x, int64_t ld_x, int32_t nx,
               const pgnn_fc_layer *front_layers, int32_t n_front,
               const float *residual, int64_t ld_res, float *y, int64_t ld_y,
               Plan &pf, FrontArgs &f) {
  PGNN_REQUIRE(x && y && nx > 0 && ld_x >= nx, PGNN_E_INVALID,
               "fused vertex stage: bad front input");
  int rc = make_plan(front_layers, n_front, nx, pf);
  if (rc) return rc;
  const int nt_last = pf.chain.l[n_front - 1].nt;
  PGNN_REQUIRE(nt_last <= kMaxTilesPerPass, PGNN_E_UNSUPPORTED,
               "fused vertex stage: front chain wider than 320");
  PGNN_REQUIRE(ld_y >= 16 * nt_last && (!residual || ld_res >= 16 * nt_last),
               PGNN_E_INVALID,
               "fused vertex stage: ld_y / ld_res < padded front width");
  f.x = x;
  f.ldx = ld_x;
  f.nx = nx;
  f.res = residual;
  f.ldres = ld_res;
  f.y = y;
  f.ldy = ld_y;
  f.ld_buf = pf.tile_floats_per_row;
  f.ld_stage = lds_ld(16 * nt_last);
  f.ts = (long long *)g_mlp_ts;
  return 0;
}

int update_pre_edge_impl(
    const float *x, int64_t ld_x, int32_t nx, const pgnn_fc_layer *front_layers,
    int32_t n_front, const float *residual, int64_t ld_res, float *y,
    int64_t ld_y, int32_t c, const float *xyz,
    const pgnn_fc_layer *offset_layers, int32_t n_offset_layers,
    const pgnn_fc_layer *p_layer, const float *wx, int64_t n_vertices, float *P,
    float *Q, int64_t ld_pq, float *agg, int64_t ld_agg, hipStream_t stream,
    const Dyn &dk) {
  PGNN_REQUIRE(n_vertices >= 0 && c > 0 && n_offset_layers >= 0 &&
                   n_offset_layers <= PGNN_MAX_LAYERS && p_layer,
               PGNN_E_INVALID, "vertex_update_pre_edge: bad argument");
  if (n_vertices == 0) return 0;
  PGNN_REQUIRE(xyz && wx && P && Q && (!agg || ld_agg > 0) && agg != x,
               PGNN_E_INVALID, "vertex_update_pre_edge: null / aliased pointer");
  PGNN_REQUIRE(expected(dk, n_vertices) <= 32 * (int64_t)device_cu_count(),
               PGNN_E_UNSUPPORTED, "vertex_update_pre_edge: too many rows");
  Plan pf;
  FrontArgs f;
  int rc = plan_front(x, ld_x, nx, front_layers, n_front, residual, ld_res, y,
                      ld_y, pf, f);
  if (rc) return rc;
  PGNN_REQUIRE(16 * pf.chain.l[n_front - 1].nt >= c &&
                   16 * pf.chain.l[n_front - 1].nt < c + 16,
               PGNN_E_INVALID,
               "vertex_update_pre_edge: front chain must produce c features");
  ChainDev off;
  LayerDev pl;
  PreEdgeArgs a;
  rc = plan_pre_edge("vertex_update_pre_edge", c, xyz, offset_layers,
                     n_offset_layers, p_layer, wx, n_vertices, P, Q, ld_pq, agg,
                     ld_agg, dk, kMaxTilesPerPass, off, pl, a);
  if (rc) return rc;
  a.h = nullptr;
  a.ld_h = 0;
  if (f.ld_buf < a.ld_tile) f.ld_buf = a.ld_tile;
  if (f.ld_stage < lds_ld(16 * pl.nt)) f.ld_stage = lds_ld(16 * pl.nt);
  const size_t lds = (size_t)16 * (f.ld_buf + a.ld_scratch + f.ld_stage) * 4;
  PGNN_REQUIRE(lds <= 160 * 1024, PGNN_E_UNSUPPORTED,
               "vertex_update_pre_edge: layers too wide for the LDS tile");
  return launch_lds(dk.dev ? vertex_update_pre_edge_kernel<true>
                           : vertex_update_pre_edge_kernel<false>,
                    dim3((unsigned)dyn_grid_tiles(dk, n_vertices)),
                    dim3(64 * kRowsWaves), lds, stream, pf.chain, f, off, pl, a);
}

int mlp2_impl(const float *x, int64_t ld_x, int32_t nx,
              const pgnn_fc_layer *front_layers, int32_t n_front,
              const float *residual, int64_t ld_res, float *y, int64_t ld_y,
              int32_t ny, const pgnn_fc_layer *back_layers, int32_t n_back,
              float *out, int64_t ld_out, int64_t n_rows, hipStream_t stream,
              const Dyn &dk) {
  PGNN_REQUIRE(n_rows >= 0 && ny > 0, PGNN_E_INVALID, "mlp2: bad sizes");
  if (n_rows == 0) return 0;
  PGNN_REQUIRE(out, PGNN_E_INVALID, "mlp2: null output");
  PGNN_REQUIRE(expected(dk, n_rows) <= 32 * (int64_t)device_cu_count(),
               PGNN_E_UNSUPPORTED, "mlp2: too many rows for the 16-row kernel");
  Plan pf;
  FrontArgs f;
  int rc = plan_front(x, ld_x, nx, front_layers, n_front, residual, ld_res, y,
                      ld_y, pf, f);
  if (rc) return rc;
  PGNN_REQUIRE(ny <= 16 * pf.chain.l[n_front - 1].nt, PGNN_E_INVALID,
               "mlp2: ny wider than the front chain's output");
  Plan pb;
  rc = make_plan(back_layers, n_back, ny, pb);
  if (rc) return rc;
  const int nt_out = pb.chain.l[n_back - 1].nt;
  PGNN_REQUIRE(nt_out <= kMaxTilesPerPass &&
                   pb.chain.l[0].kq <= kMaxTilesPerPass,
               PGNN_E_UNSUPPORTED, "mlp2: back chain wider than 320");
  PGNN_REQUIRE(ld_out >= 16 * nt_out, PGNN_E_INVALID,
               "mlp2: ld_out < padded output width");
  if (f.ld_buf < pb.tile_floats_per_row) f.ld_buf = pb.tile_floats_per_row;
  if (f.ld_stage < lds_ld(16 * nt_out)) f.ld_stage = lds_ld(16 * nt_out);
  RowsArgs ro = {};
  ro.nx = ny;
  ro.y = out;
  ro.ldy = ld_out;
  const size_t lds = (size_t)16 * (f.ld_buf + f.ld_stage) * 4;
  PGNN_REQUIRE(lds <= 160 * 1024, PGNN_E_UNSUPPORTED,
               "mlp2: layers too wide for the LDS tile");
  return launch_lds(dk.dev ? vertex_mlp2_kernel<true> : vertex_mlp2_kernel<false>,
                    dim3((unsigned)dyn_grid_tiles(dk, n_rows)),
                    dim3(64 * kRowsWaves), lds, stream, pf.chain, f, pb.chain,
                    ro, n_rows, dk.dev);
}
}

extern "C" int pgnn_vertex_update_pre_edge_fwd(
    const float *x, int64_t ld_x, int32_t nx, const pgnn_fc_layer *front_layers,
    int32_t n_front, const float *residual, int64_t ld_res, float *y,
    int64_t ld_y, int32_t c, const float *xyz,
    const pgnn_fc_layer *offset_layers, int32_t n_offset_layers,
    const pgnn_fc_layer *p_layer, const float *wx, int64_t n_vertices, float *P,
    float *Q, int64_t ld_pq, float *agg, int64_t ld_agg, void *stream_) {
  PGNN_GUARD_BEGIN
  return update_pre_edge_impl(x, ld_x, nx, front_layers, n_front, residual,
                              ld_res, y, ld_y, c, xyz, offset_layers,
                              n_offset_layers, p_layer, wx, n_vertices, P, Q,
                              ld_pq, agg, ld_agg, (hipStream_t)stream_,
                              dyn_of(nullptr));
  PGNN_GUARD_END
}

extern "C" int pgnn_vertex_update_pre_edge_fwd_dyn(
    const float *x, int64_t ld_x, int32_t nx, const pgnn_fc_layer *front_layers,
    int32_t n_front, const float *residual, int64_t ld_res, float *y,
    int64_t ld_y, int32_t c, const float *xyz,
    const pgnn_fc_layer *offset_layers, int32_t n_offset_layers,
    const pgnn_fc_layer *p_layer, const float *wx, int64_t vertices_cap,
    float *P, float *Q, int64_t ld_pq, float *agg, int64_t ld_agg,
    const pgnn_dyn_count *n_vertices, void *stream_) {
  PGNN_GUARD_BEGIN
  PGNN_REQUIRE(n_vertices && n_vertices->dev, PGNN_E_INVALID,
               "vertex_update_pre_edge_dyn: null count");
  return update_pre_edge_impl(x, ld_x, nx, front_layers, n_front, residual,
                              ld_res, y, ld_y, c, xyz, offset_layers,
                              n_offset_layers, p_layer, wx, vertices_cap, P, Q,
                              ld_pq, agg, ld_agg, (hipStream_t)stream_,
                              dyn_of(n_vertices));
  PGNN_GUARD_END
}

extern "C" int pgnn_mlp2_fwd(const float *x, int64_t ld_x, int32_t nx,
                             const pgnn_fc_layer *front_layers, int32_t n_front,
                             const float *residual, int64_t ld_res, float *y,
                             int64_t ld_y, int32_t ny,
                             const pgnn_fc_layer *back_layers, int32_t n_back,
                             float *out, int64_t ld_out, int64_t n_rows,
                             void *stream_) {
  PGNN_GUARD_BEGIN
  return mlp2_impl(x, ld_x, nx, front_layers, n_front, residual, ld_res, y,
                   ld_y, ny, back_layers, n_back, out, ld_out, n_rows,
                   (hipStream_t)stream_, dyn_of(nullptr));
  PGNN_GUARD_END
}

extern "C" int pgnn_mlp2_fwd_dyn(const float *x, int64_t ld_x, int32_t nx,
                                 const pgnn_fc_layer *front_layers,
                                 int32_t n_front, const float *residual,
                                 int64_t ld_res, float *y, int64_t ld_y,
                                 int32_t ny, const pgnn_fc_layer *back_layers,
                                 int32_t n_back, float *out, int64_t ld_out,
                                 int64_t rows_cap, const pgnn_dyn_count *rows,
                                 void *stream_) {
  PGNN_GUARD_BEGIN
  PGNN_REQUIRE(rows && rows->dev, PGNN_E_INVALID, "mlp2_dyn: null count");
  return mlp2_impl(x, ld_x, nx, front_layers, n_front, residual, ld_res, y,
                   ld_y, ny, back_layers, n_back, out, ld_out, rows_cap,
                   (hipStream_t)stream_, dyn_of(rows));
  PGNN_GUARD_END
}

extern "C" int pgnn_vertex_pre_edge_fwd(
    const float *h, int64_t ld_h, int32_t c, const float *xyz,
    const pgnn_fc_layer *offset_layers, int32_t n_offset_layers,
    const pgnn_fc_layer *p_layer, const float *wx, int64_t n_vertices, float *P,
    float *Q, int64_t ld_pq, float *agg, int64_t ld_agg, void *stream_) {
  PGNN_GUARD_BEGIN
  return pre_edge_impl(h, ld_h, c, xyz, offset_layers, n_offset_layers, p_layer,
                       wx, n_vertices, P, Q, ld_pq, agg, ld_agg,
                       (hipStream_t)stream_, dyn_of(nullptr));
  PGNN_GUARD_END
}

extern "C" int pgnn_vertex_pre_edge_fwd_dyn(
    const float *h, int64_t ld_h, int32_t c, const float *xyz,
    const pgnn_fc_layer *offset_layers, int32_t n_offset_layers,
    const pgnn_fc_layer *p_layer, const float *wx, int64_t vertices_cap,
    float *P, float *Q, int64_t ld_pq, float *agg, int64_t ld_agg,
    const pgnn_dyn_count *n_vertices, void *stream_) {
  PGNN_GUARD_BEGIN
  PGNN_REQUIRE(n_vertices && n_vertices->dev, PGNN_E_INVALID,
               "vertex_pre_edge_dyn: null count");
  return pre_edge_impl(h, ld_h, c, xyz, offset_layers, n_offset_layers, p_layer,
                       wx, vertices_cap, P, Q, ld_pq, agg, ld_agg,
                       (hipStream_t)stream_, dyn_of(n_vertices));
  PGNN_GUARD_END
}

extern "C" int pgnn_point_set_pooling_rows_fwd(
    const float *point_features, int32_t n_feat, const float *point_xyz,
    const int32_t *keypoint_indices, const int32_t *edges, int64_t n_edges,
    int32_t num_keypoints, const pgnn_fc_layer *layers, int32_t n_layers,
    int32_t edges_sorted, float *out, int64_t ld_out, float *const *acts_host,
    int64_t ld_last, void *stream_) {
  PGNN_GUARD_BEGIN
  hipStream_t stream = (hipStream_t)stream_;
  PGNN_REQUIRE(n_edges >= 0 && num_keypoints >= 0 && n_feat >= 0 && n_feat <= 13 &&
                   layers && acts_host,
               PGNN_E_INVALID, "point_set_pooling_rows: bad sizes");
  if (n_layers != 4) return PGNN_E_UNSUPPORTED;
  Plan p;
  int rc = make_plan(layers, n_layers, n_feat + 3, p);
  if (rc) return rc;
  const int out_cols = 16 * p.chain.l[n_layers - 1].nt;
  PGNN_REQUIRE(out && ld_out >= out_cols && ld_last >= out_cols && ld_last % 4 == 0,
               PGNN_E_INVALID, "point_set_pooling_rows: bad output");
  const int cus = ws_cus(stream);
  if (n_edges == 0 || num_keypoints == 0 || !pool_ws_applies(p, n_edges, cus))
    return PGNN_E_UNSUPPORTED;
  PGNN_REQUIRE(point_xyz && keypoint_indices && edges && (n_feat == 0 || point_features),
               PGNN_E_INVALID, "point_set_pooling_rows: null input");
  for (int i = 0; i < 4; ++i)
    PGNN_REQUIRE(acts_host[i] && (uintptr_t)acts_host[i] % 16 == 0, PGNN_E_INVALID,
                 "point_set_pooling_rows: activation buffers must be 16-byte "
                 "aligned");
  if (!(edges_sorted & 2)) {
    rc = fill_lowest(out, (int64_t)num_keypoints * ld_out, stream);
    if (rc) return rc;
  }
  PoolArgs pa = {point_features, n_feat, point_xyz, keypoint_indices, edges};
  SegArgs sa = {out, ld_out, num_keypoints, edges_sorted & 1};
  return launch_pool_ws(p, pa, n_edges, sa, cus, nullptr, stream, acts_host,
                        ld_last);
  PGNN_GUARD_END
}

extern "C" int pgnn_edge_mlp_scatter_max_rows_fwd(
    const float *P, const float *Q, int64_t ld_pq, int32_t width,
    const int32_t *edges, int64_t n_edges, int32_t num_vertices,
    const pgnn_fc_layer *layer, int32_t edges_sorted, float *out, int64_t ld_out,
    float *rows_out, int64_t ld_rows, float *h1_out, void *stream_) {
  PGNN_GUARD_BEGIN
  hipStream_t stream = (hipStream_t)stream_;
  PGNN_REQUIRE(n_edges >= 0 && num_vertices >= 0 && width > 0 && layer,
               PGNN_E_INVALID, "edge_mlp_rows: bad sizes");
  Plan p;
  int rc = make_plan(layer, 1, width, p);
  if (rc) return rc;
  PGNN_REQUIRE(ld_pq == 16 * p.chain.l[0].kq, PGNN_E_INVALID,
               "edge_mlp_rows: ld_pq must equal the padded width");
  const int out_cols = 16 * p.chain.l[0].nt;
  PGNN_REQUIRE(out && ld_out >= out_cols && rows_out && ld_rows >= out_cols &&
                   ld_rows % 4 == 0 && (uintptr_t)rows_out % 16 == 0,
               PGNN_E_INVALID, "edge_mlp_rows: bad output");
  const int cus = ws_cus(stream);
  if (n_edges == 0 || num_vertices == 0 || !edge_ws_applies(p, n_edges, cus))
    return PGNN_E_UNSUPPORTED;
  PGNN_REQUIRE(P && Q && edges, PGNN_E_INVALID, "edge_mlp_rows: null input");
  PGNN_REQUIRE(((uintptr_t)P % 16 == 0) && ((uintptr_t)Q % 16 == 0) &&
                   ((uintptr_t)h1_out % 16 == 0),
               PGNN_E_INVALID, "edge_mlp_rows: P/Q/H1 must be 16-byte aligned");
  if (!(edges_sorted & 2)) {
    rc = fill_lowest(out, (int64_t)num_vertices * ld_out, stream);
    if (rc) return rc;
  }
  EdgeArgs ea = {P, Q, ld_pq, edges};
  SegArgs sa = {out, ld_out, num_vertices, edges_sorted & 1};
  if (p.chain.l[0].nt == 19)
    return launch_edge_ws<19, 7>(p.chain.l[0], ea, n_edges, sa, cus, nullptr,
                                 stream, rows_out, ld_rows, h1_out);
  return launch_edge_ws<16, 8>(p.chain.l[0], ea, n_edges, sa, cus, nullptr, stream,
                               rows_out, ld_rows, h1_out);
  PGNN_GUARD_END
}

extern "C" int pgnn_offset_apply(const float *xyz, const float *delta,
                                 int64_t ld_delta, int64_t n_rows,
                                 const float *wx, float *xyz_out, float *Q,
// ... 16 lines not shown
```

point-gnn_amd/csrc/mlp_engine.h:

```cpp
#pragma once
#include "pgnn_common.h"

namespace pgnn {

#ifndef PGNN_PF4
#define PGNN_PF4 2
#endif
#ifndef PGNN_PF1
#define PGNN_PF1 4
#endif

typedef float v4f __attribute__((ext_vector_type(4)));

struct LayerDev {
  const float *wp;
  int kq;
  int nt;
  int relu_from;
};

struct ChainDev {
  int n;
  LayerDev l[PGNN_MAX_LAYERS];
};
// ... 508 lines not shown
      out[t0 + j] = (v4f){0.f, 0.f, 0.f, 0.f};
      w[0][j] = wp[(size_t)(t0 + j) * 64];
    }
#pragma unroll
    for (int q = 0; q < KQ; ++q) {
      if (q + 1 < KQ) {
#pragma unroll
        for (int j = 0; j < TB; ++j)
          w[(q + 1) & 1][j] = wp[((size_t)(q + 1) * NT + t0 + j) * 64];
      }
#pragma unroll
      for (int s = 0; s < 4; ++s)
#pragma unroll
        for (int j = 0; j < TB; ++j)
          out[t0 + j] = __builtin_amdgcn_mfma_f32_16x16x4f32(
              w[q & 1][j][s], in[q][s], out[t0 + j], 0, 0, 0);
      __builtin_amdgcn_sched_barrier(0);
    }
#pragma unroll
    for (int j = 0; j < TB; ++j) {
      const int t = t0 + j;
      const v4f b = *reinterpret_cast<const v4f *>(bias + 16 * t + g4);
#pragma unroll
      for (int r = 0; r < 4; ++r) {
        float v = out[t][r] + b[r];
        if (16 * t + g4 + r >= L.relu_from) v = v > 0.0f ? v : 0.0f;
        out[t][r] = v;
      }
    }
  }
}

template <int KQ, int... NTS>
struct RegChain;

template <int KQ>
struct RegChain<KQ> {
  static __device__ __forceinline__ void run(const ChainDev &, int, int lane,
                                             const v4f (&in)[KQ],
                                             float *__restrict__ rows16,
                                             int ld) {
    float *o = rows16 + (lane & 15) * ld + 4 * (lane >> 4);
#pragma unroll
    for (int q = 0; q < KQ; ++q) *reinterpret_cast<v4f *>(o + 16 * q) = in[q];
  }
};

template <int KQ, int NT, int... REST>
struct RegChain<KQ, NT, REST...> {
  static __device__ __forceinline__ void run(const ChainDev &chain, int li,
                                             int lane, const v4f (&in)[KQ],
                                             float *__restrict__ rows16,
                                             int ld) {
    v4f out[NT];
    reg_layer<KQ, NT>(chain.l[li], lane, in, out);
    RegChain<NT, REST...>::run(chain, li + 1, lane, out, rows16, ld);
  }
};

template <int MSUB, int NT, bool TRANSPOSED, int NW = 4>
__device__ __forceinline__ void layer_pass(const float *in, int ld_in, float *out,
                                           int ld_out, const LayerDev &L, int t0,
                                           int wave, int lane, bool skip_gemm) {
  static_assert(!TRANSPOSED || NW == 4, "transposed stage is 4-wave only");
  v4f acc[MSUB][NT];
  if (!skip_gemm) {
    gemm_tile<MSUB, NT, NW>(in, ld_in, L, t0, wave, lane, acc);
  } else {
#pragma unroll
    for (int m = 0; m < MSUB; ++m)
#pragma unroll
      for (int j = 0; j < NT; ++j) acc[m][j] = (v4f){0.f, 0.f, 0.f, 0.f};
  }
  __syncthreads();
  if constexpr (TRANSPOSED)
    store_acc_T<MSUB, NT>(out, L, t0, wave, lane, acc);
  else
    store_acc<MSUB, NT, NW>(out, ld_out, L, t0, wave, lane, acc);
  __syncthreads();
}

constexpr int kKrowNT = 3;

struct KrowPre {
  v4f b[PGNN_PF1][kKrowNT];
  float bias[kKrowNT];
};

__device__ __forceinline__ void krow_prefetch_w(const LayerDev &L, int t0,
                                                int wave, int lane,
                                                KrowPre &p) {
  const v4f *__restrict__ wp = reinterpret_cast<const v4f *>(L.wp) + lane;
  const int qstride = L.nt * 64;
#pragma unroll
  for (int j = 0; j < kKrowNT; ++j) {
    int t = t0 + wave + 8 * j;
    if (t > L.nt - 1) t = L.nt - 1;
#pragma unroll
    for (int st = 0; st < PGNN_PF1; ++st) {
      const int q = st < L.kq ? st : L.kq - 1;
      p.b[st][j] = wp[(size_t)q * qstride + t * 64];
    }
  }
}

__device__ __forceinline__ void krow_prefetch_bias(const LayerDev &L, int t0,
                                                   int wave, int lane,
                                                   KrowPre &p) {
  const float *__restrict__ bias = L.wp + (size_t)L.kq * L.nt * 256;
#pragma unroll
  for (int j = 0; j < kKrowNT; ++j) {
    int t = t0 + wave + 8 * j;
    if (t > L.nt - 1) t = L.nt - 1;
    p.bias[j] = bias[t * 16 + (lane & 15)];
  }
}

__device__ __forceinline__ void krow_prefetch(const LayerDev &L, int t0, int wave,
                                              int lane, KrowPre &p) {
  krow_prefetch_w(L, t0, wave, lane, p);
  krow_prefetch_bias(L, t0, wave, lane, p);
}

template <int NT>
__device__ __forceinline__ void layer_pass_krow(const float *in, int ld_in,
                                                float *out, int ld_out,
                                                const LayerDev &L, int t0,
                                                int wave, int lane, KrowPre &pre,
                                                bool has_next,
                                                const LayerDev next,
                                                int next_t0) {
  constexpr int PF = PGNN_PF1, NW = 8;
  static_assert(NT <= kKrowNT, "prefetch slots");
  if constexpr (NT == 0) {
    if (has_next) krow_prefetch_w(next, next_t0, wave, lane, pre);
    __syncthreads();
    if (has_next) krow_prefetch_bias(next, next_t0, wave, lane, pre);
    __syncthreads();
    return;
  } else {
  v4f acc[NT];
  int toff[NT];
#pragma unroll
  for (int j = 0; j < NT; ++j) {
    acc[j] = (v4f){0.f, 0.f, 0.f, 0.f};
    int t = t0 + wave + NW * j;
    if (t > L.nt - 1) t = L.nt - 1;
    toff[j] = t * 64;
  }
  const v4f *__restrict__ wp = reinterpret_cast<const v4f *>(L.wp) + lane;
  const float *arow = in + (lane & 15) * ld_in + 4 * (lane >> 4);
  const int qstride = L.nt * 64;
  const int kq = L.kq;
  v4f a[PF];
#pragma unroll
  for (int st = 0; st < PF; ++st)
    a[st] = *reinterpret_cast<const v4f *>(arow + 16 * (st < kq ? st : kq - 1));
  int q = 0;
  for (; q + PF <= kq; q += PF) {
#pragma unroll
    for (int st = 0; st < PF; ++st) {
#pragma unroll
      for (int s = 0; s < 4; ++s)
#pragma unroll
        for (int j = 0; j < NT; ++j)
          acc[j] = __builtin_amdgcn_mfma_f32_16x16x4f32(
              a[st][s], pre.b[st][j][s], acc[j], 0, 0, 0);
      int qn = q + st + PF;
      if (qn > kq - 1) qn = kq - 1;
#pragma unroll
      for (int j = 0; j < NT; ++j)
        pre.b[st][j] = wp[(size_t)qn * qstride + toff[j]];
      a[st] = *reinterpret_cast<const v4f *>(arow + 16 * qn);
    }
  }
  const int rem = kq - q;
#pragma unroll
  for (int st = 0; st + 1 < PF; ++st) {
    if (st < rem) {
#pragma unroll
      for (int s = 0; s < 4; ++s)
#pragma unroll
        for (int j = 0; j < NT; ++j)
          acc[j] = __builtin_amdgcn_mfma_f32_16x16x4f32(
              a[st][s], pre.b[st][j][s], acc[j], 0, 0, 0);
    }
  }
  if (has_next) krow_prefetch_w(next, next_t0, wave, lane, pre);
  __syncthreads();
#pragma unroll
  for (int j = 0; j < NT; ++j) {
    const int t = t0 + wave + NW * j;
    if (t < L.nt && t - t0 < kMaxTilesPerPass) {
      const int col = t * 16 + (lane & 15);
      const bool relu = col >= L.relu_from;
      const float bv = pre.bias[j];
      float *o = out + (4 * (lane >> 4)) * ld_out + (col - 16 * t0);
#pragma unroll
      for (int r = 0; r < 4; ++r) {
        float v = acc[j][r] + bv;
        if (relu) v = v > 0.0f ? v : 0.0f;
        o[r * ld_out] = v;
      }
    }
  }
  if (has_next) krow_prefetch_bias(next, next_t0, wave, lane, pre);
  __syncthreads();
  }
}

__device__ __forceinline__ void krow_pass(const float *in, int ld_in, float *out,
                                          int ld_out, const LayerDev &L, int t0,
                                          int wave, int lane, KrowPre &pre,
                                          bool has_next, const LayerDev next,
                                          int next_t0) {
  int tiles = L.nt - t0;
  if (tiles > kMaxTilesPerPass) tiles = kMaxTilesPerPass;
  const int ntw = tiles / 8 + (wave < tiles % 8 ? 1 : 0);
  switch (ntw) {
    case 0: layer_pass_krow<0>(in, ld_in, out, ld_out, L, t0, wave, lane, pre, has_next, next, next_t0); break;
    case 1: layer_pass_krow<1>(in, ld_in, out, ld_out, L, t0, wave, lane, pre, has_next, next, next_t0); break;
    case 2: layer_pass_krow<2>(in, ld_in, out, ld_out, L, t0, wave, lane, pre, has_next, next, next_t0); break;
    default: layer_pass_krow<3>(in, ld_in, out, ld_out, L, t0, wave, lane, pre, has_next, next, next_t0); break;
  }
}

template <int MSUB, bool TRANSPOSED, int NW = 4>
__device__ __forceinline__ void layer_pass_dispatch(const float *in, int ld_in,
                                                    float *out, int ld_out,
                                                    const LayerDev &L, int t0,
                                                    int wave, int lane,
                                                    bool skip_gemm = false) {
  int tiles = L.nt - t0;
  if (tiles > kMaxTilesPerPass) tiles = kMaxTilesPerPass;
  if constexpr (MSUB == 4 && NW == 4) {
    if (use_split(MSUB, tiles) && !skip_gemm) {
      layer_pass_split<4, 3, TRANSPOSED>(in, ld_in, out, ld_out, L, t0, wave,
                                         lane);
      return;
    }
  }
  const int ntw = (tiles + NW - 1) / NW;
  switch (ntw) {
    case 1: layer_pass<MSUB, 1, TRANSPOSED, NW>(in, ld_in, out, ld_out, L, t0, wave, lane, skip_gemm); break;
    case 2: layer_pass<MSUB, 2, TRANSPOSED, NW>(in, ld_in, out, ld_out, L, t0, wave, lane, skip_gemm); break;
    case 3: layer_pass<MSUB, 3, TRANSPOSED, NW>(in, ld_in, out, ld_out, L, t0, wave, lane, skip_gemm); break;
    case 4: layer_pass<MSUB, 4, TRANSPOSED, NW>(in, ld_in, out, ld_out, L, t0, wave, lane, skip_gemm); break;
    default: layer_pass<MSUB, 5, TRANSPOSED, NW>(in, ld_in, out, ld_out, L, t0, wave, lane, skip_gemm); break;
  }
}

}
```

point-gnn_amd/csrc/train.hip:

```cpp
#include "mlp_engine.h"
#include "sort.h"

namespace {
using namespace pgnn;

__global__ void pack_fc_device_kernel(const float *__restrict__ w,
                                      const float *__restrict__ b, int k_in,
                                      int n_out, int transpose,
                                      float *__restrict__ packed) {
  const int K = transpose ? n_out : k_in, N = transpose ? k_in : n_out;
  const int kq = (K + 15) / 16, nt = (N + 15) / 16;
  const int64_t total = (int64_t)kq * nt * 256;
  for (int64_t idx = (int64_t)blockIdx.x * blockDim.x + threadIdx.x;
       idx < total + nt * 16; idx += (int64_t)gridDim.x * blockDim.x) {
    if (idx >= total) {
      const int n = (int)(idx - total);
      packed[idx] = (!transpose && b && n < N) ? b[n] : 0.0f;
      continue;
    }
    const int s = (int)(idx & 3), lane = (int)((idx >> 2) & 63);
    const int64_t qt = idx >> 8;
    const int t = (int)(qt % nt), q = (int)(qt / nt);
    const int k = 16 * q + 4 * (lane >> 4) + s, n = 16 * t + (lane & 15);
    float v = 0.0f;
// ... 1420 lines not shown
                                      float *F, void *stream_) {
  PGNN_GUARD_BEGIN
  PGNN_REQUIRE(n_feat >= 0 && n_feat <= 13 && n_edges >= 0, PGNN_E_INVALID,
               "pool_features: bad sizes");
  if (n_edges == 0) return 0;
  PGNN_REQUIRE(point_xyz && keypoint_indices && edges && F, PGNN_E_INVALID,
               "pool_features: null pointer");
  hipLaunchKernelGGL(pool_features_wide_kernel, dim3(grid_for(n_edges * 16, 8192)),
                     dim3(256), 0, (hipStream_t)stream_, point_features,
                     (int64_t)n_feat, n_feat, point_xyz, keypoint_indices, edges,
                     n_edges, F, 16);
  PGNN_HIP(hipGetLastError());
  return 0;
  PGNN_GUARD_END
}

extern "C" int pgnn_pool_features_wide_fwd(
    const float *point_features, int64_t ld_features, int32_t n_feat,
    const float *point_xyz, const int32_t *keypoint_indices,
    const int32_t *edges, int64_t n_edges, float *F, int64_t ld_f,
    void *stream_) {
  PGNN_GUARD_BEGIN
  PGNN_REQUIRE(n_feat >= 0 && n_feat <= 4093 && ld_features >= n_feat &&
                   ld_f >= n_feat + 3 && ld_f <= 4096 && n_edges >= 0,
               PGNN_E_INVALID, "pool_features_wide: bad sizes");
  if (n_edges == 0) return 0;
  PGNN_REQUIRE((point_features || n_feat == 0) && point_xyz &&
                   keypoint_indices && edges && F,
               PGNN_E_INVALID, "pool_features_wide: null pointer");
  hipLaunchKernelGGL(pool_features_wide_kernel,
                     dim3(grid_for(n_edges * ld_f, 8192)), dim3(256), 0,
                     (hipStream_t)stream_, point_features, ld_features, n_feat,
                     point_xyz, keypoint_indices, edges, n_edges, F, (int)ld_f);
  PGNN_HIP(hipGetLastError());
  return 0;
  PGNN_GUARD_END
}

namespace {
constexpr int kMergeJobs = 48;
struct MergeJobsDev {
  pgnn_merge_job j[kMergeJobs];
  int n;
};
__global__ void merge_rows_kernel(MergeJobsDev js) {
  const pgnn_merge_job &job = js.j[blockIdx.y];
  const int32_t *src = (const int32_t *)job.src;
  int32_t *dst = (int32_t *)job.dst;
  const int32_t a0 = job.add0, a1 = job.add1;
  for (int64_t i = (int64_t)blockIdx.x * blockDim.x + threadIdx.x;
       i < job.n_words; i += (int64_t)gridDim.x * blockDim.x)
    dst[i] = src[i] + ((i & 1) ? a1 : a0);
}
}

extern "C" int pgnn_merge_rows(const pgnn_merge_job *jobs_host, int32_t n_jobs,
                               void *stream_) {
  PGNN_GUARD_BEGIN
  hipStream_t stream = (hipStream_t)stream_;
  PGNN_REQUIRE(n_jobs >= 0 && (n_jobs == 0 || jobs_host), PGNN_E_INVALID,
               "merge_rows: bad argument");
  for (int first = 0; first < n_jobs; first += kMergeJobs) {
    MergeJobsDev js;
    js.n = 0;
    int64_t longest = 0;
    for (int i = first; i < n_jobs && js.n < kMergeJobs; ++i) {
      const pgnn_merge_job &j = jobs_host[i];
      PGNN_REQUIRE(j.n_words >= 0 && (j.n_words == 0 || (j.src && j.dst)),
                   PGNN_E_INVALID, "merge_rows: bad job");
      if (j.n_words == 0) continue;
      js.j[js.n++] = j;
      if (j.n_words > longest) longest = j.n_words;
    }
    if (js.n == 0) continue;
    hipLaunchKernelGGL(merge_rows_kernel,
                       dim3(grid_for(longest, 256), (unsigned)js.n), dim3(256), 0,
                       stream, js);
  }
  PGNN_HIP(hipGetLastError());
  return 0;
  PGNN_GUARD_END
}

extern "C" int pgnn_relu_mask_mul(float *dY, const float *Y, int64_t count,
                                  void *stream_) {
  PGNN_GUARD_BEGIN
  if (count <= 0) return 0;
  PGNN_REQUIRE(dY && Y, PGNN_E_INVALID, "relu_mask_mul: null pointer");
  hipLaunchKernelGGL(relu_mask_mul_kernel, dim3(grid_for(count, 8192)),
                     dim3(256), 0, (hipStream_t)stream_, dY, Y, count);
  PGNN_HIP(hipGetLastError());
  return 0;
  PGNN_GUARD_END
}

extern "C" int pgnn_scatter_max_bwd_f32(
    const float *data, int64_t ld_data, const int32_t *seg_ids, int64_t n_rows,
    int32_t n_cols, int32_t num_segments, const float *out, int64_t ld_out,
    const float *grad_out, int64_t ld_grad_out, int32_t *tie_count_ws,
    float *grad_data, int64_t ld_grad_data, int32_t relu_mask, void *stream_) {
  PGNN_GUARD_BEGIN
  hipStream_t stream = (hipStream_t)stream_;
  PGNN_REQUIRE(n_rows >= 0 && n_cols > 0 && num_segments >= 0, PGNN_E_INVALID,
               "scatter_max_bwd: bad sizes");
  if (n_rows == 0) return 0;
  PGNN_REQUIRE(data && seg_ids && out && grad_out && tie_count_ws && grad_data,
               PGNN_E_INVALID, "scatter_max_bwd: null pointer");
  PGNN_HIP(hipMemsetAsync(tie_count_ws, 0, (size_t)num_segments * n_cols * 4,
                          stream));
  const bool vec4 =
      n_cols % 4 == 0 && ld_data % 4 == 0 && ld_out % 4 == 0 &&
      ld_grad_data % 4 == 0 && (uintptr_t)data % 16 == 0 &&
      (uintptr_t)out % 16 == 0 && (uintptr_t)grad_data % 16 == 0;
  if (vec4) {
    const unsigned g4 = grid_for(n_rows * (n_cols / 4), 8192);
    hipLaunchKernelGGL(segmax_count4_kernel, dim3(g4), dim3(256), 0, stream,
                       data, ld_data, seg_ids, n_rows, n_cols / 4, num_segments,
                       out, ld_out, tie_count_ws, relu_mask);
    hipLaunchKernelGGL(segmax_route4_kernel, dim3(g4), dim3(256), 0, stream,
                       data, ld_data, seg_ids, n_rows, n_cols / 4, num_segments,
                       out, ld_out, grad_out, ld_grad_out, tie_count_ws,
                       grad_data, ld_grad_data, relu_mask);
    PGNN_HIP(hipGetLastError());
    return 0;
  }
  const unsigned g = grid_for(n_rows * n_cols, 8192);
  hipLaunchKernelGGL(segmax_count_kernel, dim3(g), dim3(256), 0, stream, data,
                     ld_data, seg_ids, n_rows, n_cols, num_segments, out, ld_out,
                     tie_count_ws, relu_mask);
  hipLaunchKernelGGL(segmax_route_kernel, dim3(g), dim3(256), 0, stream, data,
                     ld_data, seg_ids, n_rows, n_cols, num_segments, out, ld_out,
                     grad_out, ld_grad_out, tie_count_ws, grad_data,
                     ld_grad_data, relu_mask);
  PGNN_HIP(hipGetLastError());
  return 0;
  PGNN_GUARD_END
}

namespace pgnn {
int g_wgrad_wg_target = 512;
}

namespace {
int wg_slices(int64_t rows, int k_in) {
  const int64_t in_blocks = ((int64_t)k_in + 1 + 63) / 64;
  int64_t s = (rows + kWgRows - 1) / kWgRows;
  int64_t cap = g_wgrad_wg_target / in_blocks;
  if (cap < 1) cap = 1;
  if (s > cap) s = cap;
  if (s < 1) s = 1;
  return (int)s;
}
}

extern "C" size_t pgnn_weight_grad_workspace_bytes(int32_t k_in, int32_t n_out,
                                                   int64_t n_rows) {
  if (k_in <= 0 || n_out <= 0 || n_rows < 0) return 0;
  const size_t in_blocks = ((size_t)k_in + 1 + 63) / 64;
  const size_t nt = ((size_t)n_out + 15) / 16;
  return (size_t)wg_slices(n_rows, k_in) * (in_blocks * 64 + 1) * nt * 16 * 4 +
         256;
}

extern "C" int pgnn_weight_grad_f32(const float *X, int64_t ld_x, int32_t k_in,
                                    const float *dZ, int64_t ld_dz,
                                    int32_t n_out, int64_t n_rows, float *dW,
// ... 702 lines not shown
```

point-gnn_amd/engine.py:

```python
import time

import torch

from . import graph_gen, models

__all__ = ["InferenceEngine", "DeferredFrame", "CapturedFrame", "shard_frames",
           "concurrent_streams"]

_CONCURRENT = {}


def _shares_queue(busy, cand, scratch, spin_cycles):
    with torch.cuda.stream(busy):
        torch.cuda._sleep(spin_cycles)
    ev = torch.cuda.Event()
    with torch.cuda.stream(cand):
        scratch.add_(1)
        ev.record()
    t0 = time.perf_counter()
    ev.synchronize()
    waited = time.perf_counter() - t0
    busy.synchronize()
    return waited


def concurrent_streams(n, device=None):
    dev = torch.device("cuda", torch.cuda.current_device()) \
        if device is None or device.index is None else device
    cur = torch.cuda.current_stream(dev)
    key = (dev.index, cur.cuda_stream)
    have = _CONCURRENT.setdefault(key, [])
    if len(have) >= n:
        return have[:n]
    scratch = torch.zeros(64, device=dev)
    e0, e1 = torch.cuda.Event(enable_timing=True), torch.cuda.Event(enable_timing=True)
    torch.cuda.synchronize(dev)
    e0.record()
    torch.cuda._sleep(1000000)
    e1.record()
    e1.synchronize()
    per_cycle = max(e0.elapsed_time(e1), 1e-3) / 1e6
    spin = int(1.5 / per_cycle)
    tried = 0
    while len(have) < n and tried < 24:
        cand = torch.cuda.Stream(device=dev)
        tried += 1
        clash = False
        for busy in [cur] + have:
            if _shares_queue(busy, cand, scratch, spin) > 0.6e-3:
                clash = True
                break
        if not clash:
            have.append(cand)
    while len(have) < n:
        have.append(torch.cuda.Stream(device=dev))
    return have[:n]


def shard_frames(num_frames, rank, world_size):
    if not (0 <= rank < world_size):
        raise ValueError("rank %d outside world of %d" % (rank, world_size))
    return list(range(rank, num_frames, world_size))


class DeferredFrame(object):

    def __init__(self, engine, xyz, intensity, logits, boxes, counts):
        self.engine = engine
        self.xyz, self.intensity = xyz, intensity
        self.logits, self.boxes = logits, boxes
        self.counts = counts
        self._out = None

    def result(self, host_counts=None):
        if self._out is not None:
            return self._out
        if host_counts is not None:
            self.counts._host = [int(v) for v in host_counts]
        c = self.counts
        eng = self.engine
        graph_gen.check_kd_status(c.kd_status)
        k, edges = c.k, c.edges
        eng._hints = (eng._hints or graph_gen.CountHints()).update(k, edges)
        if c.overflowed:
            eng.deferred_overflows += 1
            self._out = eng.run_frame(self.xyz, self.intensity)
        else:
            eng.frame_shapes.append((k,) + tuple(edges))
            self._out = (self.logits[:k], self.boxes[:k])
        return self._out


class CapturedFrame(object):

    def __init__(self, engine, graph, stream, xyz, intensity, frame):
        self.engine, self.graph, self.stream = engine, graph, stream
        self.xyz, self.intensity, self.frame = xyz, intensity, frame

    def replay(self, xyz, intensity):
        if tuple(xyz.shape) != tuple(self.xyz.shape) or \
                tuple(intensity.shape) != tuple(self.intensity.shape):
            raise ValueError(
                "captured for clouds of %d points, got %d: the point count "
                "shapes the kd-tree launches, capture one graph per count"
                % (self.xyz.shape[0], xyz.shape[0]))
        cur = torch.cuda.current_stream()
        self.stream.wait_stream(cur)
        with torch.cuda.stream(self.stream):
            self.xyz.copy_(xyz, non_blocking=True)
            self.intensity.copy_(intensity, non_blocking=True)
            self.graph.replay()
        cur.wait_stream(self.stream)
        f = self.frame
        out = DeferredFrame(self.engine, xyz, intensity, f.logits, f.boxes,
                            graph_gen.FrameCounts(f.counts.tensor,
                                                  f.counts.edge_caps))
        return out


class InferenceEngine(object):
    def __init__(self, config, params, box_encoding_len=7, device=None,
                 edge_arith='f32'):
        self.config = config
        self.model = models.get_model(config['model_name'])(
            num_classes=config['num_classes'],
            box_encoding_len=box_encoding_len, mode='test',
            **config['model_kwargs'])
        self.model.edge_arith = edge_arith
        self.model.load_state_dict(params, device)
        self.graph_fn = graph_gen.get_graph_generate_fn(
            config['graph_gen_method'])
        self.graph_kwargs = config['runtime_graph_gen_kwargs']
        self.time_dict = {}
        self.last_graph = None
        self.frame_shapes = []
        self._hints = None
        self.deferred_overflows = 0

    def _note_shape(self, graph):
        coords, _, edges = graph
        shape = (int(coords[1].shape[0]),) + tuple(int(e.shape[0])
                                                   for e in edges)
        self.frame_shapes.append(shape)
        self._hints = (self._hints or graph_gen.CountHints()).update(
            shape[0], shape[1:])

    def build_graph_deferred(self, xyz, overlap=False):
        if self._hints is None:
            raise RuntimeError("no size hints yet: run one frame through "
                               "run_frame() first")
        return self.graph_fn(xyz, deferred_counts=self._hints,
                             overlap_build=overlap, **self.graph_kwargs)

    def run_frame_deferred(self, xyz, intensity, overlap_build=False):
        if self._hints is None or int(xyz.shape[0]) == 0:
            out = self.run_frame(xyz, intensity)
            f = DeferredFrame(self, xyz, intensity, None, None, None)
            f._out = out
            return f
        graph = self.build_graph_deferred(xyz, overlap_build)
        coords, kps, edges = graph
        logits, boxes = self.model.predict(intensity, coords, kps, edges,
                                           is_training=False)
        self.last_graph = graph
        return DeferredFrame(self, xyz, intensity, logits, boxes,
                             edges[0]._pgnn_count.frame)

    def build_graph(self, xyz):
        return self.graph_fn(xyz, **self.graph_kwargs)

    def _pipeline_streams(self, graph_cus):
        dev_index = torch.cuda.current_device()
        key = (dev_index, int(graph_cus))
        cache = self.__dict__.setdefault("_stream_sets", {})
        if key in cache:
            return cache[key]
        graph_cus = int(graph_cus)
        if graph_cus <= 0:
            streams = list(concurrent_streams(3))
            streams += [torch.cuda.Stream() for _ in range(2)]
            cache[key] = (streams[0], streams[1:])
            return cache[key]
        import ctypes
        from . import _lib
        lib = _lib.load()
        dev = torch.device("cuda", dev_index)
        owned = self.__dict__.setdefault("_owned_streams", [])

        def make(complement):
            p = ctypes.c_void_p()
            _lib.check(lib.pgnn_stream_create_cu_mask(
                0, graph_cus, complement, ctypes.byref(p)),
                "pgnn_stream_create_cu_mask")
            owned.append(p.value)
            return torch.cuda.ExternalStream(p.value, device=dev)
        sg, aux = make(0), make(0)
        graph_gen._AUX_STREAMS[(dev.index, sg.cuda_stream)] = aux
        cache[key] = (sg, [make(1) for _ in range(4)])
        return cache[key]

    def close(self):
        owned = self.__dict__.pop("_owned_streams", [])
        self.__dict__.pop("_stream_sets", None)
        if owned:
            from . import _lib
            for k in [k for k, s in graph_gen._AUX_STREAMS.items()
                      if s.cuda_stream in owned or k[1] in owned]:
                del graph_gen._AUX_STREAMS[k]
            for k in [k for k in _lib._SCHED_WS if k[1] in owned]:
                del _lib._SCHED_WS[k]
            torch.cuda.synchronize()
            torch.cuda.empty_cache()
            lib = _lib.load()
            for h in owned:
                _lib.check(lib.pgnn_stream_destroy(h), "pgnn_stream_destroy")

    def _builder_streams(self, n, compute):
        sg, _ = self._pipeline_streams(0)
        out = [sg]
        for s in concurrent_streams(1 + len(compute) + n):
            if len(out) >= n:
                break
            if s is not sg and all(s is not c for c in compute):
                out.append(s)
        return out

    def capture_frame(self, xyz, intensity, overlap_build=False):
        if self._hints is None:
            self.run_frame(xyz, intensity)
            self.frame_shapes.pop()
        key = ("capture", torch.cuda.current_device())
        cache = self.__dict__.setdefault("_stream_sets", {})
        side = cache.get(key)
        if side is None:
            side = cache[key] = torch.cuda.Stream()
        side.wait_stream(torch.cuda.current_stream())
        with torch.cuda.stream(side):
            for _ in range(2):
                self.run_frame_deferred(xyz, intensity,
                                        overlap_build).result()
                self.frame_shapes.pop()
        torch.cuda.current_stream().wait_stream(side)
        torch.cuda.synchronize()
        xs, fs = xyz.clone(), intensity.clone()
        graph = torch.cuda.CUDAGraph()
        with torch.cuda.graph(graph, stream=side):
            frame = self.run_frame_deferred(xs, fs, overlap_build)
        torch.cuda.synchronize()
        return CapturedFrame(self, graph, side, xs, fs, frame)

    def run_frames_on_streams(self, frames, n_streams=3, gnn_priority=False):
        frames = list(frames)
        if not frames:
            return []
        if self._hints is None or not getattr(self, "_warm", False):
            self.run_frame(*frames[0])
            self.frame_shapes.pop()
            self._warm = True
        streams = list(concurrent_streams(max(1, int(n_streams))))
        cur = torch.cuda.current_stream()
        for s in streams:
            s.wait_stream(cur)
        pending = []
        t_enq = time.perf_counter()
        if gnn_priority:
            hi = self._priority_streams(len(streams))
            for h in hi:
                h.wait_stream(cur)
            for i, (xyz, intensity) in enumerate(frames):
                b, h = streams[i % len(streams)], hi[i % len(streams)]
                if int(gnn_priority) < 0:
                    b, h = h, b
                if self._hints is None or int(xyz.shape[0]) == 0:
                    with torch.cuda.stream(b):
                        pending.append(self.run_frame_deferred(xyz, intensity))
                    continue
                with torch.cuda.stream(b):
                    graph = self.build_graph_deferred(xyz)
                h.wait_stream(b)
                coords, kps, edges = graph
                with torch.cuda.stream(h):
                    for t in list(coords) + list(kps) + list(edges):
                        t.record_stream(h)
                    frame = edges[0]._pgnn_count.frame
                    frame.tensor.record_stream(h)
                    logits, boxes = self.model.predict(
                        intensity, coords, kps, edges, is_training=False)
                b.wait_stream(h)
                self.last_graph = graph
                pending.append(DeferredFrame(self, xyz, intensity, logits,
                                             boxes, frame))
            for h in hi:
                cur.wait_stream(h)
        else:
            for i, (xyz, intensity) in enumerate(frames):
                with torch.cuda.stream(streams[i % len(streams)]):
                    pending.append(self.run_frame_deferred(xyz, intensity))
        for s in streams:
            cur.wait_stream(s)
        self.last_enqueue_s = time.perf_counter() - t_enq
        live = [f for f in pending if f.counts is not None]
        host = torch.stack([f.counts.tensor for f in live]).tolist() \
            if live else []
        for f, h in zip(live, host):
            f.result(h)
        outs = [f.result() for f in pending]
        for lg, bx in outs:
            lg.record_stream(cur)
            bx.record_stream(cur)
        if not self._edge_range_clean():
            return self._rerun_batch_f32(
                lambda: self.run_frames_on_streams(frames, n_streams,
                                                   gnn_priority))
        return outs

    def _priority_streams(self, n):
        key = ("hi", torch.cuda.current_device())
        cache = self.__dict__.setdefault("_stream_sets", {})
        have = cache.setdefault(key, [])
        while len(have) < n:
            have.append(torch.cuda.Stream(priority=-1))
        return have[:n]

    def run_frames_pipelined(self, frames, compute_streams=1, graph_cus=0,
                             lookahead=0, deferred=False, graph_streams=1):
        frames = list(frames)
        if not frames:
            return []
        if not getattr(self, "_warm", False):
            self.run_frame(*frames[0])
            self.frame_shapes.pop()
            self._warm = True
        sg, scs = self._pipeline_streams(graph_cus)
        scs = scs[:max(1, min(4, int(compute_streams)))]
        sgs = [sg]
        if deferred and graph_cus <= 0 and int(graph_streams) > 1:
            sgs = self._builder_streams(int(graph_streams), scs)
        cur = torch.cuda.current_stream()
        for s in tuple(sgs) + tuple(scs):
            s.wait_stream(cur)

        def build(i):
            s_build = sgs[i % len(sgs)]
            with torch.cuda.stream(s_build):
                g = self.build_graph_deferred(frames[i][0]) if deferred \
                    else self.build_graph(frames[i][0])
                ev = torch.cuda.Event()
                ev.record(s_build)
            return g, ev

        ready = None
        worker = None
        if lookahead > 0 and len(frames) > 1:
            import queue
            import threading
            ready = queue.Queue(maxsize=int(lookahead))
            dev_index = torch.cuda.current_device()

            def produce():
                try:
                    torch.cuda.set_device(dev_index)
                    for j in range(len(frames)):
                        ready.put(build(j))
                except BaseException as exc:
                    ready.put(exc)
            worker = threading.Thread(target=produce, daemon=True)
            worker.start()

        ahead = len(sgs)
        queued = []

        def next_graph(i):
            if ready is None:
                while len(queued) < ahead and i + len(queued) < len(frames):
                    queued.append(build(i + len(queued)))
                return queued.pop(0)
            item = ready.get()
            if isinstance(item, BaseException):
                raise item
            return item

        outs = []
        try:
            graph, ev = next_graph(0)
            for i in range(len(frames)):
                sc = scs[i % len(scs)]
                sc.wait_event(ev)
                with torch.cuda.stream(sc):
                    coords, kps, edges = graph
                    for t in list(coords) + list(kps) + list(edges):
                        t.record_stream(sc)
                    if deferred:
                        counts = edges[0]._pgnn_count.frame
                        counts.tensor.record_stream(sc)
                    out = self.model.predict(frames[i][1], coords, kps,
                                             edges, is_training=False)
# ... 75 lines not shown
```

point-gnn_amd/graph_gen.py:

```python
import ctypes
import threading
import weakref

import numpy as np
import torch

from . import _lib

__all__ = ["gen_disjointed_rnn_local_graph_v3",
           "gen_multi_level_local_graph_v3", "get_graph_generate_fn",
           "multi_layer_downsampling_select", "multi_layer_downsampling_random",
           "gen_multi_level_local_graph_v3_one_read",
           "CountHints", "FrameCounts"]


class CountHints(object):

    MIN_EDGE_CAP = 1 << 16

    def __init__(self, k=0, edges=(), edge_caps=(), raw_caps=()):
        self.k = int(k)
        self.edges = [int(e) for e in edges]
        self.edge_caps = [int(c) for c in edge_caps]
        self.raw_caps = [int(c) for c in raw_caps]

    def _grown(self, caps, sizes):
        caps = list(caps) + [0] * (len(sizes) - len(caps))
        return [max(c, self.MIN_EDGE_CAP, 2 * int(e) + 1024)
                for c, e in zip(caps, sizes)]

    def update(self, k, edges, raw_edges=None):
        self.k = int(k)
        self.edges = [int(e) for e in edges]
        self.edge_caps = self._grown(self.edge_caps, edges)
        if raw_edges is not None:
            self.raw_caps = self._grown(self.raw_caps, raw_edges)
        return self

    def raw_cap(self, level):
        if level < len(self.raw_caps) and self.raw_caps[level] > 0:
            return self.raw_caps[level]
        return 2 * self.cap(level)

    def cap(self, level):
        if level < len(self.edge_caps) and self.edge_caps[level] > 0:
            return self.edge_caps[level]
        return self.MIN_EDGE_CAP

    def edge_hint(self, level):
        return self.edges[level] if level < len(self.edges) else 0


class FrameCounts(object):

    def __init__(self, tensor, edge_caps):
        self.tensor = tensor
        self.edge_caps = list(edge_caps)
        self._host = None

    def read(self):
        if self._host is None:
            self._host = [int(v) for v in self.tensor.tolist()]
        return self._host

    @property
    def k(self):
        return self.read()[0]

    @property
    def kd_status(self):
        return self.read()[1]

    @property
    def edges(self):
        v = self.read()
        return [v[3 + 2 * l] for l in range(len(self.edge_caps))]

    @property
    def raw_edges(self):
        v = self.read()
        n = len(self.edge_caps)
        if len(v) < 2 + 4 * n:
            return None
        return [v[3 + 2 * n + 2 * l] for l in range(n)]

    @property
    def overflowed(self):
        v = self.read()
        return [l for l in range(len(self.edge_caps))
                if v[3 + 2 * l] > v[2 + 2 * l]]


class _ZeroPool(object):
    kRecords, kInts = 512, 16

    class _Segment(object):
# ... 580 lines not shown
        if cfg['graph_gen_method'] != 'disjointed_rnn_local_graph_v3':
            raise NotImplementedError(
                "deferred_counts: generator %r has no capacity form"
                % (cfg['graph_gen_method'],))
    n_levels = len(level_configs)
    dev = _device()
    fan_k = [int(cfg['graph_gen_kwargs'].get('num_neighbors', -1) or -1)
             if cfg['graph_gen_kwargs'].get(
                 'neighbors_downsample_method', 'random') == 'random' else -1
             for cfg in level_configs]
    capped = any(k > 0 for k in fan_k)
    seeds = [None] * n_levels
    counts = _zero_counts(2 + (4 if capped else 2) * n_levels, dev)
    caps = [hints.cap(l) for l in range(n_levels)]
    frame = FrameCounts(counts, caps)

    def fan_in(l):
        if fan_k[l] <= 0:
            return None
        if seeds[l] is None:
            seeds[l] = int(np.random.randint(0, 2 ** 31 - 1))
        at = 2 + 2 * n_levels + 2 * l
        return (fan_k[l], seeds[l], hints.raw_cap(l), counts[at:at + 2])

    def level_job(l, points, centers_cap):
        kw = level_configs[l]['graph_gen_kwargs']
        return _RadiusDynJob(points, _lib.count_of(points), centers_cap,
                             kw['radius'], kw.get('scale'), caps[l],
                             counts[2 + 2 * l:4 + 2 * l], hints.edge_hint(l),
                             fan_in(l))

    p = _to_dev(points_xyz)[0]
    n = int(p.shape[0])
    overlap = bool(overlap) and not capped and n > 0 and \
        p.dtype == torch.float32 and n_levels >= 1 and level_configs[0]['graph_level'] == 0 and \
        not np.isclose(scales[0], 0)
    job0 = ov = None
    if overlap:
        ov = _overlap_set(dev)
        job0 = level_job(0, p, n)
        ov.fork.record()
    coords, kps, _ = _multi_layer_downsampling(
        p, base_voxel_size, scales, add_rnd3d, downsample_method,
        num_out=counts[0:2], k_hint=hints.k,
        fork_kdtree=ov.aux if overlap else False)
    if overlap:
        ov.side.wait_event(ov.fork)
        with torch.cuda.stream(ov.side):
            job0.grid()
            ov.grid.record()
    for t in list(coords) + list(kps):
        c = _lib.count_of(t)
        if c is not None:
            c.frame = frame
    edges_list = [None] * n_levels
    side_jobs = []
    if overlap:
        ov.kp.record()
        for l in range(1, n_levels):
            lvl = level_configs[l]['graph_level']
            pts, ctr = coords[lvl], coords[lvl + 1]
            side_jobs.append((l, level_job(l, pts, int(ctr.shape[0])), ctr))
        ov.side.wait_event(ov.kp)
        with torch.cuda.stream(ov.side):
            for l, job, ctr in side_jobs:
                job.grid()
                edges_list[l] = job.query(ctr, _lib.count_of(ctr))
            ov.join.record()
        torch.cuda.current_stream(dev).wait_event(ov.grid)
        edges_list[0] = job0.query(coords[1], _lib.count_of(coords[1]))
        torch.cuda.current_stream(dev).wait_event(ov.join)
    else:
        for l, cfg in enumerate(level_configs):
            lvl = cfg['graph_level']
            edges_list[l] = radius_graph_dyn_device(
                coords[lvl], coords[lvl + 1], cfg['graph_gen_kwargs']['radius'],
                cfg['graph_gen_kwargs'].get('scale'), caps[l],
                counts[2 + 2 * l:4 + 2 * l], hints.edge_hint(l), fan_in(l))
    for e in edges_list:
        _lib.count_of(e).frame = frame
    return coords, kps, edges_list


def gen_multi_level_local_graph_v3_one_read(points_xyz, hints, **kwargs):
    state = np.random.get_state()
    coords, kps, edges = gen_multi_level_local_graph_v3(
        points_xyz, deferred_counts=hints, **kwargs)
    frame = _lib.count_of(edges[0]).frame
    host = frame.read()
    check_kd_status(frame.kd_status)
    hints.update(frame.k, frame.edges, frame.raw_edges)
    if frame.overflowed:
        after = np.random.get_state()
        np.random.set_state(state)
        out = gen_multi_level_local_graph_v3(points_xyz, **kwargs)
        np.random.set_state(after)
        return out
    base = frame.tensor.storage_offset()

    def cut(t):
        c = _lib.count_of(t)
        if c is None:
            return t
        v = t[:host[c.dev.storage_offset() - base]]
        if getattr(t, '_pgnn_sorted', 0):
            v._pgnn_sorted = 1
        return v
    return [cut(t) for t in coords], [cut(t) for t in kps], \
        [cut(t) for t in edges]


def get_graph_generate_fn(method_name):
    method_map = {
        'disjointed_rnn_local_graph_v3': gen_disjointed_rnn_local_graph_v3,
        'multi_level_local_graph_v3': gen_multi_level_local_graph_v3,
    }
    return method_map[method_name]
```

Before: 318.6.

## Merge frame pairs into one GNN pass and cap waves per SIMD for strided vertex kernels

Adds a device-side merge that concatenates the point clouds, features, keypoints and edge lists of two frames with dynamic counts, so a pair of frames runs through a single GNN predict call. run_frames_on_streams now groups frames in pairs by default when the graph config allows it. This amortises per-launch and per-frame overhead and gives each launch a larger grid. Separately, the persistent-grid vertex kernels get a min-waves launch bound and a smaller prefetch depth to lower register pressure and raise occupancy. It also adds an occupancy query helper. The merge adds copy traffic and changes how results are split back per frame.

After: 326.0, median of 6. 1.02x the previous value.

```diff
diff --git a/include/pointgnn_hip.h b/include/pointgnn_hip.h
--- a/include/pointgnn_hip.h
+++ b/include/pointgnn_hip.h
@@ -425,6 +425,22 @@
 } pgnn_merge_job;
 int pgnn_merge_rows(const pgnn_merge_job *jobs_host, int32_t n_jobs,
                     void *stream);
+#define PGNN_MERGE_MAX_LEVELS 4
+typedef struct pgnn_frame_arrays {
+  int32_t *counts;
+  float *points;
+  float *features;
+  int64_t n_points;
+  float *kp_xyz;
+  int32_t *kp_idx;
+  int64_t kp_cap;
+  int32_t *edges[PGNN_MERGE_MAX_LEVELS];
+  int64_t edge_caps[PGNN_MERGE_MAX_LEVELS];
+} pgnn_frame_arrays;
+int pgnn_merge_frames_dyn(const pgnn_frame_arrays *a_host,
+                          const pgnn_frame_arrays *b_host,
+                          const pgnn_frame_arrays *merged_host, int32_t n_feat,
+                          int32_t n_levels, int64_t words_hint, void *stream);
 int pgnn_pool_features_fwd(const float *point_features, int32_t n_feat,
                            const float *point_xyz,
                            const int32_t *keypoint_indices,
@@ -714,6 +730,9 @@
     int32_t *out_count, void *stream);
 
 int pgnn_set_tunable(const char *key, int value);
+int pgnn_kernel_occupancy(const char *kernel, int64_t lds_bytes,
+                          int32_t *vgprs, int32_t *scratch_bytes,
+                          int32_t *workgroups_per_cu, int64_t *lds_used);
 int pgnn_set_debug_buffer(void *device_ptr);
 
 #ifdef __cplusplus
diff --git a/point-gnn_amd/_lib.py b/point-gnn_amd/_lib.py
--- a/point-gnn_amd/_lib.py
+++ b/point-gnn_amd/_lib.py
@@ -30,6 +30,16 @@
 class MergeJob(ctypes.Structure):
     _fields_ = [("src", c_vp), ("dst", c_vp), ("n_words", c_i64),
                 ("add0", c_i32), ("add1", c_i32)]
+
+
+MERGE_MAX_LEVELS = 4
+
+
+class FrameArrays(ctypes.Structure):
+    _fields_ = [("counts", c_vp), ("points", c_vp), ("features", c_vp),
+                ("n_points", c_i64), ("kp_xyz", c_vp), ("kp_idx", c_vp),
+                ("kp_cap", c_i64), ("edges", c_vp * MERGE_MAX_LEVELS),
+                ("edge_caps", c_i64 * MERGE_MAX_LEVELS)]
 
 
 class PackJob(ctypes.Structure):
@@ -329,6 +339,15 @@
                                        c_vp, c_vp]),
     "pgnn_relu_mask_mul": (c_i32, [c_vp, c_vp, c_i64, c_vp]),
     "pgnn_merge_rows": (c_i32, [ctypes.POINTER(MergeJob), c_i32, c_vp]),
+    "pgnn_merge_frames_dyn": (c_i32, [ctypes.POINTER(FrameArrays),
+                                      ctypes.POINTER(FrameArrays),
+                                      ctypes.POINTER(FrameArrays), c_i32,
+                                      c_i32, c_i64, c_vp]),
+    "pgnn_kernel_occupancy": (c_i32, [ctypes.c_char_p, c_i64,
+                                      ctypes.POINTER(c_i32),
+                                      ctypes.POINTER(c_i32),
+                                      ctypes.POINTER(c_i32),
+                                      ctypes.POINTER(c_i64)]),
     "pgnn_scatter_max_bwd_f32": (c_i32, [c_vp, c_i64, c_vp, c_i64, c_i32,
                                          c_i32, c_vp, c_i64, c_vp, c_i64, c_vp,
                                          c_vp, c_i64, c_i32, c_vp]),
@@ -527,5 +546,15 @@
     return getattr(t, "_pgnn_count", None) if t is not None else None
 
 
+def kernel_occupancy(kernel, lds_bytes=-1):
+    v, sc, wg = c_i32(0), c_i32(0), c_i32(0)
+    used = c_i64(0)
+    check(load().pgnn_kernel_occupancy(
+        kernel.encode(), int(lds_bytes), ctypes.byref(v), ctypes.byref(sc),
+        ctypes.byref(wg), ctypes.byref(used)), "pgnn_kernel_occupancy")
+    return {"vgprs": v.value, "scratch_bytes": sc.value,
+            "workgroups_per_cu": wg.value, "lds_bytes": used.value}
+
+
 def set_tunable(key, value):
     check(load().pgnn_set_tunable(key.encode(), int(value)), "pgnn_set_tunable")
diff --git a/point-gnn_amd/csrc/gnn.hip b/point-gnn_amd/csrc/gnn.hip
--- a/point-gnn_amd/csrc/gnn.hip
+++ b/point-gnn_amd/csrc/gnn.hip
@@ -1,3 +1,5 @@
+#include <atomic>
+
 #include "mlp_engine.h"
 #include "edge_ws.h"
 #include "edge_ws_split.h"
@@ -183,8 +185,9 @@
 __device__ __forceinline__ void consume_rows16(const float *__restrict__ stage,
                                                int ld, int64_t row0,
                                                int rows_valid, int col0,
-                                               int ncols, const RowsArgs &ra) {
-  const int r = threadIdx.x >> 5, c0 = threadIdx.x & 31;
+                                               int ncols, const RowsArgs &ra,
+                                               int tid = (int)threadIdx.x) {
+  const int r = tid >> 5, c0 = tid & 31;
   const int64_t row = row0 + (r < rows_valid ? r : rows_valid - 1);
   float add[kRowSteps];
   if (ra.res) {
@@ -245,8 +248,9 @@
 __device__ __forceinline__ void load_rows16(const float *__restrict__ x,
                                             int64_t ldx, int nx, float *tile,
                                             int ld0, int kc, int64_t row0,
-                                            int rows_valid) {
-  const int r = threadIdx.x >> 5, c0 = threadIdx.x & 31;
+                                            int rows_valid,
+                                            int tid = (int)threadIdx.x) {
+  const int r = tid >> 5, c0 = tid & 31;
   const float *__restrict__ xr =
       x + (row0 + (r < rows_valid ? r : rows_valid - 1)) * ldx;
   for (int cb = 0; cb < kc; cb += 32 * kRowSteps) {
@@ -800,6 +804,8 @@
 }
 
 constexpr int kRowsWaves = 8;
+constexpr int kRowsWavesPerSimd2 = 2 * kRowsWaves / 4;
+constexpr int kRowsPf2 = PGNN_PF1 < 3 ? PGNN_PF1 : 3;
 
 template <bool TAPS>
 __global__ __launch_bounds__(64 * kRowsWaves) void rows_mlp_kernel(
@@ -1645,12 +1651,14 @@
   int ld_tile, ld_scratch;
 };
 
+template <int PF>
 __device__ __forceinline__ void pre_edge_tail(const ChainDev &off,
                                               const LayerDev &pl,
                                               const PreEdgeArgs &a, float *tile,
                                               float *scratch, float *stage,
                                               int64_t row0, int rows_valid,
-                                              int wave, int lane, KrowPre &pre) {
+                                              int wave, int lane,
+                                              KrowPreT<PF> &pre, int tid) {
   const float *delta = nullptr;
   int ld_delta = 0;
   for (int li = 0; li < off.n; ++li) {
@@ -1663,7 +1671,7 @@
     ld_delta = lds_ld(16 * L.nt);
   }
   {
-    const int r = threadIdx.x >> 5, c0 = threadIdx.x & 31;
+    const int r = tid >> 5, c0 = tid & 31;
     const int ldq = (int)a.ld_pq;
     const int64_t row = row0 + (r < rows_valid ? r : rows_valid - 1);
     float x0 = a.xyz[row * 3], x1 = a.xyz[row * 3 + 1], x2 = a.xyz[row * 3 + 2];
@@ -1694,11 +1702,11 @@
   RowsArgs ra = {};
   ra.y = a.P;
   ra.ldy = a.ld_pq;
-  consume_rows16(stage, ld_st, row0, rows_valid, 0, 16 * pl.nt, ra);
+  consume_rows16(stage, ld_st, row0, rows_valid, 0, 16 * pl.nt, ra, tid);
 }
 
 template <bool STRIDE>
-__global__ __launch_bounds__(64 * kRowsWaves) void vertex_pre_edge_kernel(
+__global__ __launch_bounds__(64 * kRowsWaves, STRIDE ? kRowsWavesPerSimd2 : 1) void vertex_pre_edge_kernel(
     ChainDev off, LayerDev pl, PreEdgeArgs a) {
   constexpr int ROWS = 16;
   extern __shared__ __attribute__((aligned(16))) char smem[];
@@ -1715,14 +1723,15 @@
   for (int64_t row0 = (int64_t)blockIdx.x * ROWS; row0 < n_rows;
        row0 += STRIDE ? (int64_t)gridDim.x * ROWS : n_rows) {
     const int lane = opaque_lane(lane_id);
+    const int tid = STRIDE ? opaque_lane(threadIdx.x) : (int)threadIdx.x;
   const int rows_valid =
       (int)((n_rows - row0 < ROWS) ? (n_rows - row0) : ROWS);
   const int kc = 16 * pl.kq;
-  KrowPre pre;
+  KrowPreT<STRIDE ? kRowsPf2 : PGNN_PF1> pre;
   krow_prefetch(off.n > 0 ? off.l[0] : pl, 0, wave, lane, pre);
   {
     static_assert(64 * kRowsWaves == 32 * ROWS, "one 32-thread group per row");
-    const int r = threadIdx.x >> 5, c0 = threadIdx.x & 31;
+    const int r = tid >> 5, c0 = tid & 31;
     const int64_t rowc = row0 + (r < rows_valid ? r : rows_valid - 1);
     const float *__restrict__ hr = a.h + rowc * a.ld_h;
     const float *__restrict__ xr = a.xyz + rowc * 3;
@@ -1746,12 +1755,12 @@
     }
   }
   if (a.agg) {
-    for (int idx = threadIdx.x; idx < rows_valid * (int)a.ld_agg; idx += 64 * kRowsWaves)
+    for (int idx = tid; idx < rows_valid * (int)a.ld_agg; idx += 64 * kRowsWaves)
       a.agg[row0 * a.ld_agg + idx] = kFloatLowest;
   }
   __syncthreads();
   pre_edge_tail(off, pl, a, tile, scratch, stage, row0, rows_valid, wave, lane,
-                pre);
+                pre, tid);
   if (STRIDE) __syncthreads();
   }
 }
@@ -1769,9 +1778,11 @@
   long long *ts;
 };
 
+template <int PF>
 __device__ __forceinline__ void front_chain(const ChainDev &front, float *tile,
                                             float *stage, int ld_stage,
-                                            int wave, int lane, KrowPre &pre,
+                                            int wave, int lane,
+                                            KrowPreT<PF> &pre,
                                             const LayerDev after,
                                             long long *tsw, int &n_stamp) {
   for (int li = 0; li + 1 < front.n; ++li) {
@@ -1790,7 +1801,7 @@
 }
 
 template <bool STRIDE>
-__global__ __launch_bounds__(64 * kRowsWaves) void vertex_update_pre_edge_kernel(
+__global__ __launch_bounds__(64 * kRowsWaves, STRIDE ? kRowsWavesPerSimd2 : 1) void vertex_update_pre_edge_kernel(
     ChainDev front, FrontArgs f, ChainDev off, LayerDev pl, PreEdgeArgs a) {
   constexpr int ROWS = 16;
   static_assert(64 * kRowsWaves == 32 * ROWS, "one 32-thread group per row");
@@ -1823,14 +1834,15 @@
   for (int64_t row0 = (int64_t)blockIdx.x * ROWS; row0 < n_rows;
        row0 += STRIDE ? (int64_t)gridDim.x * ROWS : n_rows) {
     const int lane = opaque_lane(lane_id);
+    const int tid = STRIDE ? opaque_lane(threadIdx.x) : (int)threadIdx.x;
     const int rows_valid =
         (int)((n_rows - row0 < ROWS) ? (n_rows - row0) : ROWS);
     stamp();
-    KrowPre pre;
+    KrowPreT<STRIDE ? kRowsPf2 : PGNN_PF1> pre;
     krow_prefetch(front.l[0], 0, wave, lane, pre);
-    load_rows16(f.x, f.ldx, f.nx, tile, lds_ld(kc0), kc0, row0, rows_valid);
+    load_rows16(f.x, f.ldx, f.nx, tile, lds_ld(kc0), kc0, row0, rows_valid, tid);
     if (a.agg) {
-      for (int idx = threadIdx.x; idx < rows_valid * (int)a.ld_agg;
+      for (int idx = tid; idx < rows_valid * (int)a.ld_agg;
            idx += 64 * kRowsWaves)
         a.agg[row0 * a.ld_agg + idx] = kFloatLowest;
     }
@@ -1840,7 +1852,7 @@
                 off.n > 0 ? off.l[0] : pl, tsw, n_stamp);
     stamp();
     {
-      const int r = threadIdx.x >> 5, c0 = threadIdx.x & 31;
+      const int r = tid >> 5, c0 = tid & 31;
       const int64_t row = row0 + (r < rows_valid ? r : rows_valid - 1);
       float add[kRowSteps];
       if (f.res) {
@@ -1876,7 +1888,7 @@
     __syncthreads();
     stamp();
     pre_edge_tail(off, pl, a, tile, scratch, stage, row0, rows_valid, wave, lane,
-                  pre);
+                  pre, tid);
     stamp();
     if (STRIDE) __syncthreads();
   }
@@ -1884,7 +1896,7 @@
 }
 
 template <bool STRIDE>
-__global__ __launch_bounds__(64 * kRowsWaves) void vertex_mlp2_kernel(
+__global__ __launch_bounds__(64 * kRowsWaves, STRIDE ? kRowsWavesPerSimd2 : 1) void vertex_mlp2_kernel(
     ChainDev front, FrontArgs f, ChainDev back, RowsArgs out, int64_t n_rows,
     const int32_t *n_dev) {
   constexpr int ROWS = 16;
@@ -1904,18 +1916,19 @@
   for (int64_t row0 = (int64_t)blockIdx.x * ROWS; row0 < n_rows;
        row0 += STRIDE ? (int64_t)gridDim.x * ROWS : n_rows) {
     const int lane = opaque_lane(lane_id);
+    const int tid = STRIDE ? opaque_lane(threadIdx.x) : (int)threadIdx.x;
     const int rows_valid =
         (int)((n_rows - row0 < ROWS) ? (n_rows - row0) : ROWS);
-    KrowPre pre;
+    KrowPreT<STRIDE ? kRowsPf2 : PGNN_PF1> pre;
     krow_prefetch(front.l[0], 0, wave, lane, pre);
-    load_rows16(f.x, f.ldx, f.nx, tile, lds_ld(kc0), kc0, row0, rows_valid);
+    load_rows16(f.x, f.ldx, f.nx, tile, lds_ld(kc0), kc0, row0, rows_valid, tid);
     __syncthreads();
     int no_stamp = 0;
     front_chain(front, tile, stage, f.ld_stage, wave, lane, pre, back.l[0],
                 nullptr, no_stamp);
     const int kmax = kcb > ncols_y ? kcb : ncols_y;
     {
-      const int r = threadIdx.x >> 5, c0 = threadIdx.x & 31;
+      const int r = tid >> 5, c0 = tid & 31;
       const int64_t row = row0 + (r < rows_valid ? r : rows_valid - 1);
       float add[kRowSteps];
       if (f.res) {
@@ -1952,7 +1965,7 @@
     const int ld_st = lds_ld(16 * L.nt);
     krow_pass(tile, lds_ld(16 * L.kq), stage, ld_st, L, 0, wave, lane, pre,
               false, L, 0);
-    consume_rows16(stage, ld_st, row0, rows_valid, 0, 16 * L.nt, out);
+    consume_rows16(stage, ld_st, row0, rows_valid, 0, 16 * L.nt, out, tid);
     if (STRIDE) __syncthreads();
   }
 }
@@ -1960,6 +1973,8 @@
 }
 
 namespace {
+std::atomic<int64_t> g_vertex_lds[3][2] = {{{-1}, {-1}}, {{-1}, {-1}}, {{-1}, {-1}}};
+
 int plan_pre_edge(const char *name, int32_t c, const float *xyz,
                   const pgnn_fc_layer *offset_layers, int32_t n_offset_layers,
                   const pgnn_fc_layer *p_layer, const float *wx,
@@ -2037,6 +2052,7 @@
       (size_t)16 * (a.ld_tile + a.ld_scratch + lds_ld(16 * pl.nt)) * 4;
   PGNN_REQUIRE(lds <= 160 * 1024, PGNN_E_UNSUPPORTED,
                "vertex_pre_edge: layer too wide for the LDS tile");
+  g_vertex_lds[0][dk.dev ? 1 : 0] = (int64_t)lds;
   return launch_lds(
       dk.dev ? vertex_pre_edge_kernel<true> : vertex_pre_edge_kernel<false>,
       dim3((unsigned)dyn_grid_tiles(dk, n_vertices)), dim3(64 * kRowsWaves), lds,
@@ -2111,6 +2127,7 @@
   const size_t lds = (size_t)16 * (f.ld_buf + a.ld_scratch + f.ld_stage) * 4;
   PGNN_REQUIRE(lds <= 160 * 1024, PGNN_E_UNSUPPORTED,
                "vertex_update_pre_edge: layers too wide for the LDS tile");
+  g_vertex_lds[1][dk.dev ? 1 : 0] = (int64_t)lds;
   return launch_lds(dk.dev ? vertex_update_pre_edge_kernel<true>
                            : vertex_update_pre_edge_kernel<false>,
                     dim3((unsigned)dyn_grid_tiles(dk, n_vertices)),
@@ -2153,6 +2170,7 @@
   const size_t lds = (size_t)16 * (f.ld_buf + f.ld_stage) * 4;
   PGNN_REQUIRE(lds <= 160 * 1024, PGNN_E_UNSUPPORTED,
                "mlp2: layers too wide for the LDS tile");
+  g_vertex_lds[2][dk.dev ? 1 : 0] = (int64_t)lds;
   return launch_lds(dk.dev ? vertex_mlp2_kernel<true> : vertex_mlp2_kernel<false>,
                     dim3((unsigned)dyn_grid_tiles(dk, n_rows)),
                     dim3(64 * kRowsWaves), lds, stream, pf.chain, f, pb.chain,
@@ -2249,6 +2267,55 @@
   return pre_edge_impl(h, ld_h, c, xyz, offset_layers, n_offset_layers, p_layer,
                        wx, vertices_cap, P, Q, ld_pq, agg, ld_agg,
                        (hipStream_t)stream_, dyn_of(n_vertices));
+  PGNN_GUARD_END
+}
+
+extern "C" int pgnn_kernel_occupancy(const char *kernel, int64_t lds_bytes,
+                                     int32_t *vgprs, int32_t *scratch_bytes,
+                                     int32_t *workgroups_per_cu,
+                                     int64_t *lds_used) {
+  PGNN_GUARD_BEGIN
+  PGNN_REQUIRE(kernel && vgprs && scratch_bytes && workgroups_per_cu,
+               PGNN_E_INVALID, "kernel_occupancy: null argument");
+  const std::string name(kernel);
+  const struct {
+    const char *name;
+    const void *fn[2];
+  } table[3] = {
+      {"vertex_pre_edge",
+       {reinterpret_cast<const void *>(vertex_pre_edge_kernel<false>),
+        reinterpret_cast<const void *>(vertex_pre_edge_kernel<true>)}},
+      {"vertex_update_pre_edge",
+       {reinterpret_cast<const void *>(vertex_update_pre_edge_kernel<false>),
+        reinterpret_cast<const void *>(vertex_update_pre_edge_kernel<true>)}},
+      {"vertex_mlp2",
+       {reinterpret_cast<const void *>(vertex_mlp2_kernel<false>),
+        reinterpret_cast<const void *>(vertex_mlp2_kernel<true>)}},
+  };
+  for (int i = 0; i < 3; ++i)
+    for (int dyn = 0; dyn < 2; ++dyn) {
+      if (name != std::string(table[i].name) + (dyn ? "_dyn" : "")) continue;
+      if (lds_bytes < 0) lds_bytes = g_vertex_lds[i][dyn];
+      PGNN_REQUIRE(lds_bytes >= 0 && lds_bytes <= 160 * 1024, PGNN_E_INVALID,
+                   "kernel_occupancy: no launch of this kernel yet, or more "
+                   "LDS than a CU has");
+      if (lds_bytes) {
+        const int rc = ensure_dynamic_lds(table[i].fn[dyn], (size_t)lds_bytes);
+        if (rc) return rc;
+      }
+      hipFuncAttributes attr;
+      PGNN_HIP(hipFuncGetAttributes(&attr, table[i].fn[dyn]));
+      int blocks = 0;
+      PGNN_HIP(hipOccupancyMaxActiveBlocksPerMultiprocessor(
+          &blocks, table[i].fn[dyn], 64 * kRowsWaves, (size_t)lds_bytes));
+      *vgprs = attr.numRegs;
+      *scratch_bytes = (int32_t)attr.localSizeBytes;
+      *workgroups_per_cu = blocks;
+      if (lds_used) *lds_used = lds_bytes;
+      return 0;
+    }
+  PGNN_REQUIRE(false, PGNN_E_INVALID, "kernel_occupancy: unknown kernel");
+  return 0;
   PGNN_GUARD_END
 }
 
diff --git a/point-gnn_amd/csrc/mlp_engine.h b/point-gnn_amd/csrc/mlp_engine.h
--- a/point-gnn_amd/csrc/mlp_engine.h
+++ b/point-gnn_amd/csrc/mlp_engine.h
@@ -614,14 +614,17 @@
 
 constexpr int kKrowNT = 3;
 
-struct KrowPre {
-  v4f b[PGNN_PF1][kKrowNT];
+template <int PF>
+struct KrowPreT {
+  v4f b[PF][kKrowNT];
   float bias[kKrowNT];
 };
-
+using KrowPre = KrowPreT<PGNN_PF1>;
+
+template <int PF>
 __device__ __forceinline__ void krow_prefetch_w(const LayerDev &L, int t0,
                                                 int wave, int lane,
-                                                KrowPre &p) {
+                                                KrowPreT<PF> &p) {
   const v4f *__restrict__ wp = reinterpret_cast<const v4f *>(L.wp) + lane;
   const int qstride = L.nt * 64;
 #pragma unroll
@@ -629,16 +632,17 @@
     int t = t0 + wave + 8 * j;
     if (t > L.nt - 1) t = L.nt - 1;
 #pragma unroll
-    for (int st = 0; st < PGNN_PF1; ++st) {
+    for (int st = 0; st < PF; ++st) {
       const int q = st < L.kq ? st : L.kq - 1;
       p.b[st][j] = wp[(size_t)q * qstride + t * 64];
     }
   }
 }
 
+template <int PF>
 __device__ __forceinline__ void krow_prefetch_bias(const LayerDev &L, int t0,
                                                    int wave, int lane,
-                                                   KrowPre &p) {
+                                                   KrowPreT<PF> &p) {
   const float *__restrict__ bias = L.wp + (size_t)L.kq * L.nt * 256;
 #pragma unroll
   for (int j = 0; j < kKrowNT; ++j) {
@@ -648,30 +652,21 @@
   }
 }
 
+template <int PF>
 __device__ __forceinline__ void krow_prefetch(const LayerDev &L, int t0, int wave,
-                                              int lane, KrowPre &p) {
+                                              int lane, KrowPreT<PF> &p) {
   krow_prefetch_w(L, t0, wave, lane, p);
   krow_prefetch_bias(L, t0, wave, lane, p);
 }
 
-template <int NT>
-__device__ __forceinline__ void layer_pass_krow(const float *in, int ld_in,
-                                                float *out, int ld_out,
-                                                const LayerDev &L, int t0,
-                                                int wave, int lane, KrowPre &pre,
-                                                bool has_next,
-                                                const LayerDev next,
-                                                int next_t0) {
-  constexpr int PF = PGNN_PF1, NW = 8;
+template <int NT, int PF>
+__device__ __forceinline__ void krow_gemm(const float *in, int ld_in,
+                                          const LayerDev &L, int t0, int wave,
+                                          int lane, KrowPreT<PF> &pre,
+                                          v4f (&acc)[kKrowNT]) {
+  constexpr int NW = 8;
   static_assert(NT <= kKrowNT, "prefetch slots");
-  if constexpr (NT == 0) {
-    if (has_next) krow_prefetch_w(next, next_t0, wave, lane, pre);
-    __syncthreads();
-    if (has_next) krow_prefetch_bias(next, next_t0, wave, lane, pre);
-    __syncthreads();
-    return;
-  } else {
-  v4f acc[NT];
+  if constexpr (NT > 0) {
   int toff[NT];
 #pragma unroll
   for (int j = 0; j < NT; ++j) {
@@ -718,10 +713,30 @@
               a[st][s], pre.b[st][j][s], acc[j], 0, 0, 0);
     }
   }
+  }
+}
+
+template <int PF>
+__device__ __forceinline__ void krow_pass(const float *in, int ld_in, float *out,
+                                          int ld_out, const LayerDev &L, int t0,
+                                          int wave, int lane, KrowPreT<PF> &pre,
+                                          bool has_next, const LayerDev next,
+                                          int next_t0) {
+  constexpr int NW = 8;
+  int tiles = L.nt - t0;
+  if (tiles > kMaxTilesPerPass) tiles = kMaxTilesPerPass;
+  const int ntw = tiles / 8 + (wave < tiles % 8 ? 1 : 0);
+  v4f acc[kKrowNT];
+  switch (ntw) {
+    case 0: krow_gemm<0>(in, ld_in, L, t0, wave, lane, pre, acc); break;
+    case 1: krow_gemm<1>(in, ld_in, L, t0, wave, lane, pre, acc); break;
+    case 2: krow_gemm<2>(in, ld_in, L, t0, wave, lane, pre, acc); break;
+    default: krow_gemm<3>(in, ld_in, L, t0, wave, lane, pre, acc); break;
+  }
   if (has_next) krow_prefetch_w(next, next_t0, wave, lane, pre);
   __syncthreads();
 #pragma unroll
-  for (int j = 0; j < NT; ++j) {
+  for (int j = 0; j < kKrowNT; ++j) {
     const int t = t0 + wave + NW * j;
     if (t < L.nt && t - t0 < kMaxTilesPerPass) {
       const int col = t * 16 + (lane & 15);
@@ -738,23 +753,6 @@
   }
   if (has_next) krow_prefetch_bias(next, next_t0, wave, lane, pre);
   __syncthreads();
-  }
-}
-
-__device__ __forceinline__ void krow_pass(const float *in, int ld_in, float *out,
-                                          int ld_out, const LayerDev &L, int t0,
-                                          int wave, int lane, KrowPre &pre,
-                                          bool has_next, const LayerDev next,
-                                          int next_t0) {
-  int tiles = L.nt - t0;
-  if (tiles > kMaxTilesPerPass) tiles = kMaxTilesPerPass;
-  const int ntw = tiles / 8 + (wave < tiles % 8 ? 1 : 0);
-  switch (ntw) {
-    case 0: layer_pass_krow<0>(in, ld_in, out, ld_out, L, t0, wave, lane, pre, has_next, next, next_t0); break;
-    case 1: layer_pass_krow<1>(in, ld_in, out, ld_out, L, t0, wave, lane, pre, has_next, next, next_t0); break;
-    case 2: layer_pass_krow<2>(in, ld_in, out, ld_out, L, t0, wave, lane, pre, has_next, next, next_t0); break;
-    default: layer_pass_krow<3>(in, ld_in, out, ld_out, L, t0, wave, lane, pre, has_next, next, next_t0); break;
-  }
 }
 
 template <int MSUB, bool TRANSPOSED, int NW = 4>
diff --git a/point-gnn_amd/csrc/train.hip b/point-gnn_amd/csrc/train.hip
--- a/point-gnn_amd/csrc/train.hip
+++ b/point-gnn_amd/csrc/train.hip
@@ -1526,6 +1526,131 @@
   PGNN_GUARD_END
 }
 
+namespace {
+struct MergeFramesArgs {
+  pgnn_frame_arrays a, b, m;
+  int n_feat, n_levels;
+};
+
+__device__ __forceinline__ void merge_split(int64_t na, int64_t cap_a,
+                                            int64_t nb, int64_t cap_b,
+                                            int64_t cap_m, int64_t &ta,
+                                            int64_t &tb) {
+  ta = na < 0 ? 0 : (na < cap_a ? na : cap_a);
+  if (ta > cap_m) ta = cap_m;
+  tb = nb < 0 ? 0 : (nb < cap_b ? nb : cap_b);
+  if (tb > cap_m - ta) tb = cap_m - ta;
+}
+
+__global__ void merge_frames_kernel(MergeFramesArgs g) {
+  const int arr = blockIdx.y >> 1, second = blockIdx.y & 1;
+  const pgnn_frame_arrays &f = second ? g.b : g.a;
+  int64_t ka, kb;
+  merge_split(g.a.counts[0], g.a.kp_cap, g.b.counts[0], g.b.kp_cap, g.m.kp_cap,
+              ka, kb);
+  const int64_t n_a = g.a.n_points;
+  const int32_t *src = nullptr;
+  int32_t *dst = nullptr;
+  int64_t n_words = 0;
+  int32_t add0 = 0, add1 = 0;
+  if (arr == 0) {
+    src = (const int32_t *)f.points;
+    dst = (int32_t *)g.m.points + (second ? 3 * n_a : 0);
+    n_words = 3 * f.n_points;
+  } else if (arr == 1) {
+    src = (const int32_t *)f.features;
+    dst = (int32_t *)g.m.features + (second ? g.n_feat * n_a : 0);
+    n_words = (int64_t)g.n_feat * f.n_points;
+  } else if (arr == 2) {
+    src = (const int32_t *)f.kp_xyz;
+    dst = (int32_t *)g.m.kp_xyz + (second ? 3 * ka : 0);
+    n_words = 3 * (second ? kb : ka);
+  } else if (arr == 3) {
+    src = f.kp_idx;
+    dst = g.m.kp_idx + (second ? ka : 0);
+    n_words = second ? kb : ka;
+    add0 = add1 = second ? (int32_t)n_a : 0;
+  } else {
+    const int l = arr - 4;
+    int64_t ea, eb;
+    merge_split(g.a.counts[2 + 2 * l], g.a.edge_caps[l],
+                g.b.counts[2 + 2 * l], g.b.edge_caps[l], g.m.edge_caps[l], ea,
+                eb);
+    src = f.edges[l];
+    dst = g.m.edges[l] + (second ? 2 * ea : 0);
+    n_words = 2 * (second ? eb : ea);
+    if (second) {
+      add0 = l == 0 ? (int32_t)n_a : (int32_t)ka;
+      add1 = (int32_t)ka;
+    }
+    if (!second && l == 0 && blockIdx.x == 0 && threadIdx.x == 0) {
+      g.m.counts[0] = (int32_t)(ka + kb);
+      g.m.counts[1] = g.a.counts[1] ? g.a.counts[1] : g.b.counts[1];
+      for (int j = 0; j < g.n_levels; ++j) {
+        int64_t wa, wb;
+        merge_split(g.a.counts[2 + 2 * j], g.a.edge_caps[j],
+                    g.b.counts[2 + 2 * j], g.b.edge_caps[j], g.m.edge_caps[j],
+                    wa, wb);
+        g.m.counts[2 + 2 * j] = (int32_t)(wa + wb);
+        g.m.counts[3 + 2 * j] =
+            g.a.counts[3 + 2 * j] + g.b.counts[3 + 2 * j];
+      }
+    }
+  }
+  if (arr == 0 || arr == 1 || arr == 2) {
+    for (int64_t i = (int64_t)blockIdx.x * blockDim.x + threadIdx.x; i < n_words;
+         i += (int64_t)gridDim.x * blockDim.x)
+      dst[i] = src[i];
+  } else {
+    for (int64_t i = (int64_t)blockIdx.x * blockDim.x + threadIdx.x; i < n_words;
+         i += (int64_t)gridDim.x * blockDim.x)
+      dst[i] = src[i] + ((i & 1) ? add1 : add0);
+  }
+}
+}
+
+extern "C" int pgnn_merge_frames_dyn(const pgnn_frame_arrays *a,
+                                     const pgnn_frame_arrays *b,
+                                     const pgnn_frame_arrays *merged,
+                                     int32_t n_feat, int32_t n_levels,
+                                     int64_t words_hint, void *stream_) {
+  PGNN_GUARD_BEGIN
+  PGNN_REQUIRE(a && b && merged && n_feat >= 0 && n_levels >= 1 &&
+                   n_levels <= PGNN_MERGE_MAX_LEVELS,
+               PGNN_E_INVALID, "merge_frames_dyn: bad argument");
+  MergeFramesArgs g = {*a, *b, *merged, n_feat, n_levels};
+  int64_t longest = 1;
+  for (const pgnn_frame_arrays *f : {a, b}) {
+    PGNN_REQUIRE(f->counts && f->n_points > 0 && f->points &&
+                     (n_feat == 0 || f->features) && f->kp_xyz && f->kp_idx &&
+                     f->kp_cap > 0,
+                 PGNN_E_INVALID, "merge_frames_dyn: null input");
+    for (int l = 0; l < n_levels; ++l) {
+      PGNN_REQUIRE(f->edges[l] && f->edge_caps[l] > 0, PGNN_E_INVALID,
+                   "merge_frames_dyn: null edge list");
+      if (2 * f->edge_caps[l] > longest) longest = 2 * f->edge_caps[l];
+    }
+    if (f->n_points * (n_feat > 3 ? n_feat : 3) > longest)
+      longest = f->n_points * (n_feat > 3 ? n_feat : 3);
+  }
+  PGNN_REQUIRE(merged->counts && merged->points && merged->kp_xyz &&
+                   merged->kp_idx && (n_feat == 0 || merged->features) &&
+                   merged->n_points == a->n_points + b->n_points &&
+                   merged->kp_cap > 0 &&
+                   merged->n_points <= (int64_t)INT32_MAX,
+               PGNN_E_INVALID, "merge_frames_dyn: bad output");
+  for (int l = 0; l < n_levels; ++l)
+    PGNN_REQUIRE(merged->edges[l] && merged->edge_caps[l] > 0, PGNN_E_INVALID,
+                 "merge_frames_dyn: null output edge list");
+  if (words_hint > 0 && words_hint < longest) longest = words_hint;
+  hipLaunchKernelGGL(merge_frames_kernel,
+                     dim3(grid_for(longest, 1024), (unsigned)(2 * (4 + n_levels))),
+                     dim3(256), 0, (hipStream_t)stream_, g);
+  PGNN_HIP(hipGetLastError());
+  return 0;
+  PGNN_GUARD_END
+}
+
 extern "C" int pgnn_relu_mask_mul(float *dY, const float *Y, int64_t count,
                                   void *stream_) {
   PGNN_GUARD_BEGIN
diff --git a/point-gnn_amd/engine.py b/point-gnn_amd/engine.py
--- a/point-gnn_amd/engine.py
+++ b/point-gnn_amd/engine.py
@@ -65,11 +65,13 @@
 
 class DeferredFrame(object):
 
-    def __init__(self, engine, xyz, intensity, logits, boxes, counts):
+    def __init__(self, engine, xyz, intensity, logits, boxes, counts,
+                 pair=None):
         self.engine = engine
         self.xyz, self.intensity = xyz, intensity
         self.logits, self.boxes = logits, boxes
         self.counts = counts
+        self.pair = pair
         self._out = None
 
     def result(self, host_counts=None):
@@ -85,9 +87,14 @@
         if c.overflowed:
             eng.deferred_overflows += 1
             self._out = eng.run_frame(self.xyz, self.intensity)
+        elif self.pair is not None and any(p.overflowed for p in self.pair):
+            self._out = eng.run_frame(self.xyz, self.intensity)
         else:
             eng.frame_shapes.append((k,) + tuple(edges))
-            self._out = (self.logits[:k], self.boxes[:k])
+            r0 = 0
+            if self.pair is not None and self.pair[0] is not c:
+                r0 = self.pair[0].k
+            self._out = (self.logits[r0:r0 + k], self.boxes[r0:r0 + k])
         return self._out
 
 
@@ -165,6 +172,39 @@
         self.last_graph = graph
         return DeferredFrame(self, xyz, intensity, logits, boxes,
                              edges[0]._pgnn_count.frame)
+
+    def _pairs_apply(self):
+        if self._hints is None or self.model.edge_arith != 'f32' or \
+                self.graph_fn is not graph_gen.gen_multi_level_local_graph_v3:
+            return False
+        cus = torch.cuda.get_device_properties(
+            torch.cuda.current_device()).multi_processor_count
+        if 2 * self._hints.k > 32 * cus:
+            return False
+        levels = self.graph_kwargs.get('level_configs') or []
+        if not 1 <= len(levels) <= 4 or \
+                self.graph_kwargs.get('add_rnd3d', False):
+            return False
+        scales = [float(cfg['graph_scale']) for cfg in levels]
+        if abs(scales[0]) < 1e-8 or \
+                any(abs(s - scales[0]) > 1e-8 * abs(scales[0]) for s in scales):
+            return False
+        return all(
+            cfg['graph_gen_method'] == 'disjointed_rnn_local_graph_v3' and
+            int(cfg['graph_gen_kwargs'].get('num_neighbors', -1) or -1) <= 0
+            for cfg in levels)
+
+    def run_pair_deferred(self, frame_a, frame_b):
+        (xa, ia), (xb, ib) = frame_a, frame_b
+        ga = self.build_graph_deferred(xa)
+        gb = self.build_graph_deferred(xb)
+        feats, coords, kps, edges = graph_gen.merge_frames_dyn(ga, ia, gb, ib)
+        logits, boxes = self.model.predict(feats, coords, kps, edges,
+                                           is_training=False)
+        self.last_graph = gb
+        pair = (ga[2][0]._pgnn_count.frame, gb[2][0]._pgnn_count.frame)
+        return (DeferredFrame(self, xa, ia, logits, boxes, pair[0], pair),
+                DeferredFrame(self, xb, ib, logits, boxes, pair[1], pair))
 
     def build_graph(self, xyz):
         return self.graph_fn(xyz, **self.graph_kwargs)
@@ -249,7 +289,8 @@
         torch.cuda.synchronize()
         return CapturedFrame(self, graph, side, xs, fs, frame)
 
-    def run_frames_on_streams(self, frames, n_streams=3, gnn_priority=False):
+    def run_frames_on_streams(self, frames, n_streams=3, gnn_priority=False,
+                              frames_per_pass=2):
         frames = list(frames)
         if not frames:
             return []
@@ -292,6 +333,22 @@
                                              boxes, frame))
             for h in hi:
                 cur.wait_stream(h)
+        elif int(frames_per_pass) >= 2 and self._pairs_apply():
+            def pairable(fr):
+                return int(fr[0].shape[0]) > 0 and \
+                    fr[0].dtype == torch.float32 and \
+                    fr[1].dtype == torch.float32
+            for j in range((len(frames) + 1) // 2):
+                group = frames[2 * j:2 * j + 2]
+                with torch.cuda.stream(streams[j % len(streams)]):
+                    if len(group) == 2 and pairable(group[0]) and \
+                            pairable(group[1]) and \
+                            group[0][1].shape[1:] == group[1][1].shape[1:]:
+                        pending.extend(self.run_pair_deferred(*group))
+                    else:
+                        for xyz, intensity in group:
+                            pending.append(
+                                self.run_frame_deferred(xyz, intensity))
         else:
             for i, (xyz, intensity) in enumerate(frames):
                 with torch.cuda.stream(streams[i % len(streams)]):
@@ -303,7 +360,7 @@
         host = torch.stack([f.counts.tensor for f in live]).tolist() \
             if live else []
         for f, h in zip(live, host):
-            f.result(h)
+            f.counts._host = [int(v) for v in h]
         outs = [f.result() for f in pending]
         for lg, bx in outs:
             lg.record_stream(cur)
@@ -311,7 +368,8 @@
         if not self._edge_range_clean():
             return self._rerun_batch_f32(
                 lambda: self.run_frames_on_streams(frames, n_streams,
-                                                   gnn_priority))
+                                                   gnn_priority,
+                                                   frames_per_pass))
         return outs
 
     def _priority_streams(self, n):
diff --git a/point-gnn_amd/graph_gen.py b/point-gnn_amd/graph_gen.py
--- a/point-gnn_amd/graph_gen.py
+++ b/point-gnn_amd/graph_gen.py
@@ -11,7 +11,7 @@
            "gen_multi_level_local_graph_v3", "get_graph_generate_fn",
            "multi_layer_downsampling_select", "multi_layer_downsampling_random",
            "gen_multi_level_local_graph_v3_one_read",
-           "CountHints", "FrameCounts"]
+           "CountHints", "FrameCounts", "merge_frames_dyn"]
 
 
 class CountHints(object):
@@ -758,6 +758,85 @@
     return coords, kps, edges_list
 
 
+def merge_frames_dyn(graph_a, features_a, graph_b, features_b):
+    (ca, ka, ea), (cb, kb, eb) = graph_a, graph_b
+    n_levels = len(ea)
+    if n_levels != len(eb) or not 1 <= n_levels <= _lib.MERGE_MAX_LEVELS:
+        raise ValueError("merge_frames_dyn: 1..%d edge levels, the same in "
+                         "both frames" % _lib.MERGE_MAX_LEVELS)
+    recs = []
+    for coords, kps, edges in (graph_a, graph_b):
+        cnt = _lib.count_of(edges[0])
+        if cnt is None or cnt.frame is None or \
+                _lib.count_of(coords[1]) is None or \
+                any(c is not coords[1] for c in coords[2:]) or \
+                coords[0].dtype != torch.float32 or int(coords[0].shape[0]) == 0:
+            raise ValueError("merge_frames_dyn: capacity-form frames with one "
+                             "pooling level and a non-empty float32 cloud")
+        if int(cnt.frame.tensor.shape[0]) != 2 + 2 * n_levels:
+            raise ValueError("merge_frames_dyn: frames with a fan-in cap")
+        recs.append(cnt.frame)
+    fa, fb = features_a.contiguous(), features_b.contiguous()
+    n_feat = int(fa.shape[1])
+    if fa.dtype != torch.float32 or fb.dtype != torch.float32 or \
+            int(fb.shape[1]) != n_feat:
+        raise ValueError("merge_frames_dyn: float32 features of one width")
+    dev = ca[0].device
+    n_a, n_b = int(ca[0].shape[0]), int(cb[0].shape[0])
+    kp_cap = int(ca[1].shape[0]) + int(cb[1].shape[0])
+    caps = [int(ea[l].shape[0]) + int(eb[l].shape[0]) for l in range(n_levels)]
+    points = torch.empty((n_a + n_b, 3), dtype=torch.float32, device=dev)
+    feats = torch.empty((n_a + n_b, n_feat), dtype=torch.float32, device=dev)
+    kp_xyz = torch.empty((kp_cap, 3), dtype=torch.float32, device=dev)
+    kp_idx = torch.empty((kp_cap, 1), dtype=torch.int32, device=dev)
+    edges = [torch.empty((c, 2), dtype=torch.int32, device=dev) for c in caps]
+    counts = torch.empty(2 + 2 * n_levels, dtype=torch.int32, device=dev)
+
+    def arrays(rec, pts, ft, kxyz, kidx, es):
+        out = _lib.FrameArrays()
+        out.counts = rec.data_ptr()
+        out.points, out.features = pts.data_ptr(), ft.data_ptr()
+        out.n_points = int(pts.shape[0])
+        out.kp_xyz, out.kp_idx = kxyz.data_ptr(), kidx.data_ptr()
+        out.kp_cap = int(kxyz.shape[0])
+        for l, e in enumerate(es):
+            out.edges[l] = e.data_ptr()
+            out.edge_caps[l] = int(e.shape[0])
+        return out
+    ins = [(ca[0].contiguous(), ca[1].contiguous(), ka[0].contiguous(),
+            [e.contiguous() for e in ea]),
+           (cb[0].contiguous(), cb[1].contiguous(), kb[0].contiguous(),
+            [e.contiguous() for e in eb])]
+    hint_e = [[_lib.count_of(e).hint for e in es] for es in (ea, eb)]
+    hint_k = [_lib.count_of(c[1]).hint for c in (ca, cb)]
+    words = 0
+    if all(h > 0 for hs in hint_e for h in hs):
+        words = max([2 * h for hs in hint_e for h in hs] +
+                    [max(3, n_feat) * max(n_a, n_b)])
+    _lib.check(_lib.load().pgnn_merge_frames_dyn(
+        ctypes.byref(arrays(recs[0].tensor, ins[0][0], fa, ins[0][1],
+                            ins[0][2], ins[0][3])),
+        ctypes.byref(arrays(recs[1].tensor, ins[1][0], fb, ins[1][1],
+                            ins[1][2], ins[1][3])),
+        ctypes.byref(arrays(counts, points, feats, kp_xyz, kp_idx, edges)),
+        n_feat, n_levels, words, _lib.stream_ptr()), "pgnn_merge_frames_dyn")
+    frame = FrameCounts(counts, caps)
+    cnt_k = _lib.DeviceCount(counts[0:1], sum(hint_k) if all(hint_k) else 0,
+                             frame)
+    _lib.tag_count(kp_xyz, cnt_k)
+    _lib.tag_count(kp_idx, cnt_k)
+    coords = [points] + [kp_xyz] * (len(ca) - 1)
+    kps = [kp_idx] + [_lib.tag_count(_identity_indices(kp_cap, dev), cnt_k)
+                      for _ in range(len(ka) - 1)]
+    for l, e in enumerate(edges):
+        ha, hb = hint_e[0][l], hint_e[1][l]
+        _lib.tag_count(e, _lib.DeviceCount(
+            counts[2 + 2 * l:3 + 2 * l], ha + hb if ha and hb else 0, frame))
+        if all(getattr(x[l], "_pgnn_sorted", 0) for x in (ea, eb)):
+            e._pgnn_sorted = 1
+    return feats, coords, kps, edges
+
+
 def gen_multi_level_local_graph_v3_one_read(points_xyz, hints, **kwargs):
     state = np.random.get_state()
     coords, kps, edges = gen_multi_level_local_graph_v3(
```
